# jhbastek/PhysicsInformedDiffusionModels

Measured on NVIDIA H100. Metric: train samples/s Darcy 64x64 PIDM, higher is better.
Workload: dtype bf16

## Files before the change

include/pidm.h:

```cpp
#ifndef PIDM_H_
#define PIDM_H_

#ifdef __cplusplus
extern "C" {
#endif

#ifndef PIDM_F32
#define PIDM_F32 0
#define PIDM_BF16 1
#endif

const char* pidm_last_error(void);
int pidm_version(void);

int pidm_qsample(const float* x0, const float* noise, const long long* t, const float* sqrt_ab,
                 const float* sqrt_1mab, float* xt, int B, int per_sample, void* stream);
int pidm_posterior_step(const float* x_t, const float* x0_pred, const float* z, float* out, float coef1, float coef2,
                        float sigma, long long n, void* stream);
int pidm_axpby_per_sample(const float* a, const float* x, const float* b, const float* y, const float* c,
                          const float* z, float* out, int B, int per_sample, void* stream);
int pidm_ddim_coefs(const long long* t, const long long* t_next, const float* posterior_mean_coef1,
                    const float* posterior_mean_coef2, const float* sqrt_recip_alphas, const float* noise_mean_coeff,
                    const float* alphas_prod, float* coef_x0, float* coef_x, int B, void* stream);
int pidm_scale(const float* x, const float* alpha_dev, float* out, long long n, void* stream);

int pidm_toy_pidm_loss(const float* target, const float* output, const float* residual, const float* ineq,
                       const float* opt, const long long* t, const float* p2_loss_weight,
                       const float* posterior_var_clipped, float c_data, float c_residual, float c_ineq, float lambda_opt,
                       float* sums7, float* grad_output, float* grad_residual, float* grad_ineq, float* grad_opt, int B,
                       int D, void* stream);

#define PIDM_DARCY_PIXELS_AT_BOUNDARY 1
#define PIDM_DARCY_PERIODIC 2
int pidm_darcy_residual_fwd(const float* x0hat, const float* f_s, float* residual, int B, int pixels,
                            float domain_length, int reverse_d1, int flags, void* stream);
int pidm_darcy_residual_bwd(const float* x0hat, const float* f_s, const float* grad_residual, float* grad_x0hat, int B,
                            int pixels, float domain_length, int reverse_d1, int flags, void* stream);
#define PIDM_FD_PERIODIC 8
int pidm_fd_stencil(const float* u, float* out, int planes, int pixels, int mode, float d0, float d1, void* stream);
int pidm_darcy_pidm_loss(const float* x0hat, const float* model_out, const float* target, const float* f_s,
                         const long long* t, const float* p2_loss_weight, const float* posterior_var_clipped,
                         float c_data, float c_residual, float* sums3, float* grad_x0hat, float* grad_model_out, int B,
                         int pixels, float domain_length, int reverse_d1, int flags, void* stream);
int pidm_darcy_jacobian_max(const float* x0hat, float* max_dr_dp, int B, int pixels, float domain_length, int reverse_d1,
                            int flags, void* stream);

int pidm_nchw_to_nhwc(const float* src, void* dst, int B, int C, int HW, int Cpad, int dtype, void* stream);
int pidm_nhwc_to_nchw(const void* src, float* dst, int B, int C, int HW, int Cpad, int dtype, void* stream);
int pidm_add(const void* a, const void* b, void* out, long long n, int dtype, void* stream);
int pidm_gelu_fwd(const void* x, void* y, long long n, int dtype, void* stream);
int pidm_gelu_bwd(const void* x, const void* dy, void* dx, long long n, int dtype, void* stream);
int pidm_concat_channels(const void* a, const void* b, void* out, long long rows, int Ca, int Cb, int dtype, void* stream);
int pidm_split_channels(const void* g, void* ga, void* gb, long long rows, int Ca, int Cb, int dtype, void* stream);

int pidm_pack_entry_size(void);
int pidm_pack_weights(const void* table_dev, int n_entries, int dtype, void* stream);
int pidm_pack_pair_entry_size(void);
int pidm_pack_weights_pairs(const void* table_dev, const int* tile_map_dev, int tile_base, int n_tiles, int max_taps,
                            int dtype, void* stream);
int pidm_conv2d_simt(const void* x, const void* w_packed, const float* bias, const void* residual, void* y, int B,
                     int H, int W, int Cin, int Ho, int Wo, int Cout, int KH, int KW, int stride, int pad,
                     int transposed, int dtype, void* stream);
int pidm_conv2d_wgrad_simt(const void* x, const void* dy, float* dw, float* dbias, int B, int H, int W, int Cin,
                           int Cin_real, int Ho, int Wo, int Cout, int KH, int KW, int stride, int pad, int transposed,
                           long long w_stride_n, long long w_stride_c, int dtype, void* stream);
int pidm_debug_set_trace(void* buf);
int pidm_conv2d_tc_general(const void* x, const void* w_packed, const float* bias, const void* residual, void* y, int B,
                           int H, int W, int Cin, int Ho, int Wo, int Cout, int KH, int KW, int stride, int pad,
                           int transposed, float* gn_sums, int gn_groups, int gn_sums_zeroed, void* stream);
int pidm_conv2d_tc_general_supported(int B, int H, int W, int Cin, int Ho, int Wo, int Cout, int KH, int KW, int stride,
                                     int pad, int transposed);
int pidm_conv2d_tc_plan(int B, int H, int W, int Cin, int Ho, int Wo, int Cout, int KH, int KW, int stride, int pad,
                        int transposed, int* out);
int pidm_conv2d_wgrad_tc(const void* a, const void* b, float* dw, int B, int HA, int WA, int CA, int CA_real, int GH,
                         int GW, int CB, int KH, int KW, int a_stride, int pad, long long s_row, long long s_col,
                         void* stream);
int pidm_conv2d_wgrad_tc_supported(int B, int GH, int GW, int CA, int CB, int KH, int KW, int a_stride);
int pidm_conv2d_wgrad_tc_plan(int B, int HA, int WA, int CA, int CA_real, int GH, int GW, int CB, int KH, int KW,
                              int a_stride, int pad, long long s_row, long long s_col, int* out);
int pidm_colsum(const void* x, float* out, long long M, int C, int dtype, void* stream);

int pidm_groupnorm_silu_fwd(const void* x, const float* gamma, const float* beta, const float* scale_shift,
                            const void* residual, void* y, float* sums, int stats_precomputed, int B, int HW, int C, int G,
                            float eps, int dtype, void* stream);
int pidm_groupnorm_silu_bwd(const void* x, const void* dy, const float* sums, const float* gamma, const float* beta,
                            const float* scale_shift, void* dx, float* dgamma, float* dbeta, float* d_scale_shift,
                            float* dbias_of_producer, float* workspace, int B, int HW, int C, int G, float eps,
                            int dtype, void* stream);
int pidm_layernorm_c_fwd(const void* x, const float* gamma, void* y, long long M, int C, float eps, int dtype, void* stream);
int pidm_layernorm_c_bwd(const void* x, const void* dy, const float* gamma, void* dx, float* dgamma,
                         const void* dx_residual , long long M, int C,
                         float eps, int dtype, void* stream);

int pidm_linattn_fused_supported(int C, int heads, int N, int dtype);
int pidm_linattn_fused_workspace_floats(int B, int N);
int pidm_linattn_fused_plan(int B, int N, int* out);
int pidm_linattn_fused_fwd(const void* xn, const void* w_qkv, void* out, float* ctx, float* kmax, float* kzinv,
                           float* workspace, int B, int N, void* stream);
int pidm_linattn_fused_bwd(const void* xn, const void* w_qkv, const void* dout, const float* ctx, const float* kmax,
                           const float* kzinv, void* dxn, float* dctx, int B, int N, void* stream);
int pidm_linattn_fused_wgrad(const void* xn, const void* w_qkv, const void* dout, const float* ctx, const float* dctx,
                             const float* kmax, const float* kzinv, float* grad_w, int B, int N, long long w_stride_n,
                             long long w_stride_c, void* stream);
int pidm_linattn_workspace_floats(int B, int N, int heads);
int pidm_linattn_fwd(const void* qkv, void* out, float* ctx, float* kmax, float* kzinv, float* workspace, int B, int N,
                     int heads, int dtype, void* stream);
int pidm_linattn_bwd(const void* qkv, const void* dout, const float* ctx, const float* kmax, const float* kzinv,
                     void* dqkv, float* dctx_scratch, int B, int N, int heads, int dtype, void* stream);
int pidm_attn_fwd(const void* qkv, void* out, int B, int n_tokens, int heads, int dtype, void* stream);
int pidm_attn_bwd(const void* qkv, const void* dout, void* dqkv, int B, int n_tokens, int heads, int dtype, void* stream);

int pidm_time_embed_fwd(const long long* t, const float* W1, const float* b1, const float* W2, const float* b2,
                        float* emb, float* h1, float* temb, float* silu_t, int B, int dim, int td, void* stream);
int pidm_time_embed_bwd(const float* d_silu_t, const float* emb, const float* h1, const float* temb, const float* W2,
                        float* dW1, float* db1, float* dW2, float* db2, float* workspace, int B, int dim, int td,
                        int parts, void* stream);
int pidm_mlp_entry_size(void);
int pidm_block_mlps_fwd(const void* table_dev, int n_entries, int max_rows, const float* silu_t, int B, int td,
                        void* stream);
int pidm_block_mlps_bwd(const void* table_dev, int n_entries, int max_rows, const float* silu_t, float* d_silu_t, int B,
                        int td, int parts, void* stream);

int pidm_head_fwd(const void* x, const float* w, const float* bias, float* y, int B, int HW, int C, int O,
                  int sigmoid_last, int dtype, void* stream);
int pidm_head_bwd(const void* x, const float* w, const float* y, const float* dy, void* dx, float* dw, float* db, int B,
                  int HW, int C, int O, int sigmoid_last, int dtype, void* stream);

int pidm_sumsq(const float* x, long long n, float* out, float* workspace, void* stream);
int pidm_adam_ema_step(float* param, float* grad, float* exp_avg, float* exp_avg_sq, float* ema_shadow, long long n,
                       float lr, double beta1, double beta2, float eps, int step, int* step_counter_dev,
                       const float* grad_norm_sq_dev, float grad_scale, float max_norm, float ema_mu,
                       int ema_first_step, int zero_grad, void* stream);

int pidm_mechanics_residual_fwd(const float* u, const float* rho, const float* bcs, const float* KE, float* residual,
                                float* compliance, int B, int nel, void* stream);
int pidm_mechanics_residual_bwd(const float* u, const float* rho, const float* bcs, const float* KE,
                                const float* grad_residual, const float* grad_compliance, float* grad_u, float* grad_rho,
                                float* workspace , int B, int nel, void* stream);
int pidm_mech_pidm_loss(const float* u, const float* rho, const float* x0, const float* residual, const float* compliance,
                        const float* vf, const long long* t, const float* p2_loss_weight,
                        const float* posterior_var_clipped, float c_data, float c_residual, float c_ineq,
                        float lambda_opt, float* sums6, float* grad_u, float* grad_rho, float* grad_residual,
                        float* grad_compliance, int B, int nel, void* stream);
int pidm_bilinear_resize_fwd(const float* x, float* y, int planes, int in, int out, void* stream);
int pidm_bilinear_resize_bwd(const float* dy, float* dx, int planes, int in, int out, void* stream);

#ifdef __cplusplus
}
#endif
#endif
```

physicsinformeddiffusionmodels_b200/_lib.py:

```python
import ctypes
import os

import torch

_HERE = os.path.dirname(os.path.abspath(__file__))
LIB_PATH = os.path.join(_HERE, 'libpidm.so')

P = ctypes.c_void_p
I = ctypes.c_int
L = ctypes.c_longlong
F = ctypes.c_float
D = ctypes.c_double

_SIGS = {
    'pidm_qsample': [P, P, P, P, P, P, I, I, P],
    'pidm_posterior_step': [P, P, P, P, F, F, F, L, P],
    'pidm_scale': [P, P, P, L, P],
    'pidm_ddim_coefs': [P, P, P, P, P, P, P, P, P, I, P],
    'pidm_axpby_per_sample': [P, P, P, P, P, P, P, I, I, P],
    'pidm_toy_pidm_loss': [P, P, P, P, P, P, P, P, F, F, F, F, P, P, P, P, P, I, I, P],
    'pidm_fd_stencil': [P, P, I, I, I, F, F, P],
    'pidm_darcy_residual_fwd': [P, P, P, I, I, F, I, I, P],
    'pidm_darcy_residual_bwd': [P, P, P, P, I, I, F, I, I, P],
    'pidm_darcy_jacobian_max': [P, P, I, I, F, I, I, P],
    'pidm_darcy_pidm_loss': [P, P, P, P, P, P, P, F, F, P, P, P, I, I, F, I, I, P],
    'pidm_nchw_to_nhwc': [P, P, I, I, I, I, I, P],
    'pidm_nhwc_to_nchw': [P, P, I, I, I, I, I, P],
    'pidm_add': [P, P, P, L, I, P],
    'pidm_gelu_fwd': [P, P, L, I, P],
    'pidm_gelu_bwd': [P, P, P, L, I, P],
    'pidm_concat_channels': [P, P, P, L, I, I, I, P],
    'pidm_split_channels': [P, P, P, L, I, I, I, P],
    'pidm_pack_entry_size': [],
    'pidm_pack_weights': [P, I, I, P],
    'pidm_pack_pair_entry_size': [],
    'pidm_pack_weights_pairs': [P, P, I, I, I, I, P],
    'pidm_conv2d_simt': [P, P, P, P, P, I, I, I, I, I, I, I, I, I, I, I, I, I, P],
    'pidm_conv2d_wgrad_simt': [P, P, P, P, I, I, I, I, I, I, I, I, I, I, I, I, I, L, L, I, P],
    'pidm_debug_set_trace': [P],
    'pidm_conv2d_tc_general': [P, P, P, P, P, I, I, I, I, I, I, I, I, I, I, I, I, P, I, I, P],
    'pidm_conv2d_tc_general_supported': [I, I, I, I, I, I, I, I, I, I, I, I],
    'pidm_conv2d_tc_plan': [I, I, I, I, I, I, I, I, I, I, I, I, P],
    'pidm_conv2d_wgrad_tc': [P, P, P, I, I, I, I, I, I, I, I, I, I, I, I, L, L, P],
    'pidm_conv2d_wgrad_tc_supported': [I, I, I, I, I, I, I, I],
    'pidm_conv2d_wgrad_tc_plan': [I, I, I, I, I, I, I, I, I, I, I, I, L, L, P],
    'pidm_colsum': [P, P, L, I, I, P],
    'pidm_groupnorm_silu_fwd': [P, P, P, P, P, P, P, I, I, I, I, I, F, I, P],
    'pidm_groupnorm_silu_bwd': [P, P, P, P, P, P, P, P, P, P, P, P, I, I, I, I, F, I, P],
    'pidm_layernorm_c_fwd': [P, P, P, L, I, F, I, P],
    'pidm_layernorm_c_bwd': [P, P, P, P, P, P, L, I, F, I, P],
    'pidm_linattn_workspace_floats': [I, I, I],
    'pidm_linattn_fused_supported': [I, I, I, I],
    'pidm_linattn_fused_workspace_floats': [I, I],
    'pidm_linattn_fused_plan': [I, I, P],
    'pidm_linattn_fused_fwd': [P, P, P, P, P, P, P, I, I, P],
    'pidm_linattn_fused_bwd': [P, P, P, P, P, P, P, P, I, I, P],
    'pidm_linattn_fused_wgrad': [P, P, P, P, P, P, P, P, I, I, L, L, P],
    'pidm_linattn_fwd': [P, P, P, P, P, P, I, I, I, I, P],
    'pidm_linattn_bwd': [P, P, P, P, P, P, P, I, I, I, I, P],
    'pidm_attn_fwd': [P, P, I, I, I, I, P],
    'pidm_attn_bwd': [P, P, P, I, I, I, I, P],
    'pidm_time_embed_fwd': [P, P, P, P, P, P, P, P, P, I, I, I, P],
    'pidm_time_embed_bwd': [P, P, P, P, P, P, P, P, P, P, I, I, I, I, P],
    'pidm_mlp_entry_size': [],
    'pidm_block_mlps_fwd': [P, I, I, P, I, I, P],
    'pidm_block_mlps_bwd': [P, I, I, P, P, I, I, I, P],
    'pidm_head_fwd': [P, P, P, P, I, I, I, I, I, I, P],
    'pidm_head_bwd': [P, P, P, P, P, P, P, I, I, I, I, I, I, P],
    'pidm_sumsq': [P, L, P, P, P],
    'pidm_adam_ema_step': [P, P, P, P, P, L, F, D, D, F, I, P, P, F, F, F, I, I, P],
    'pidm_mechanics_residual_fwd': [P, P, P, P, P, P, I, I, P],
    'pidm_mechanics_residual_bwd': [P, P, P, P, P, P, P, P, P, I, I, P],
    'pidm_mech_pidm_loss': [P, P, P, P, P, P, P, P, P, F, F, F, F, P, P, P, P, P, I, I, P],
    'pidm_bilinear_resize_fwd': [P, P, I, I, I, P],
    'pidm_bilinear_resize_bwd': [P, P, I, I, I, P],
    'pidm_version': [],
}
_VALUE_RETURN = {'pidm_pack_entry_size', 'pidm_pack_pair_entry_size', 'pidm_mlp_entry_size', 'pidm_linattn_workspace_floats', 'pidm_version',
                 'pidm_linattn_fused_supported', 'pidm_linattn_fused_workspace_floats',
                 'pidm_conv2d_tc_supported', 'pidm_conv2d_wgrad_tc_supported', 'pidm_conv2d_tc_general_supported',
                 'pidm_conv2d_tc_plan', 'pidm_conv2d_wgrad_tc_plan', 'pidm_linattn_fused_plan'}

if not os.path.exists(LIB_PATH):
    raise ImportError(f'{LIB_PATH} is missing: build it with `python __graft_entry__.py` (nvcc, sm_90a). '
                      'There is no CPU / PyTorch fallback for the PIDM hot path.')

_lib = ctypes.CDLL(LIB_PATH)
_lib.pidm_last_error.restype = ctypes.c_char_p
_lib.pidm_last_error.argtypes = []
for _n, _a in _SIGS.items():
    _f = getattr(_lib, _n)
    _f.argtypes = _a
    _f.restype = ctypes.c_int

launch_count = 0


def exported_symbols():
    return sorted(_SIGS) + ['pidm_last_error']


def ptr(t):
    if t is None:
        return None
    return t.data_ptr()


def stream():
    return torch.cuda.current_stream().cuda_stream


def call(name, *args):
    global launch_count
    conv = []
    for a in args:
        if isinstance(a, torch.Tensor):
            conv.append(a.data_ptr())
        else:
            conv.append(a)
    rc = getattr(_lib, name)(*conv)
    if name in _VALUE_RETURN:
        return rc
    launch_count += 1
    if rc != 0:
        raise RuntimeError(f'{name} failed (code {rc}): {_lib.pidm_last_error().decode()}')
    return 0


DTYPE_CODE = {torch.float32: 0, torch.bfloat16: 1}
```

physicsinformeddiffusionmodels_b200/csrc/attention_fused.cu:

```cuda
#define PIDM_PDL_GROUP 1
#include "common.cuh"
#include "mma_util.cuh"
#include "pidm.h"

namespace pidm {

constexpr int LF_C = 32;

__device__ __forceinline__ uint32_t movm_t(uint32_t x) {
    uint32_t y;
    asm volatile("movmatrix.sync.aligned.m8n8.trans.b16 %0, %1;" : "=r"(y) : "r"(x));
    return y;
}

__device__ __forceinline__ void load_w_frags(uint32_t (&w)[2][4][2], const __nv_bfloat16* __restrict__ Wrows, int lane) {
    const int g = lane >> 2, t = lane & 3;
#pragma unroll
    for (int ks = 0; ks < 2; ++ks)
#pragma unroll
        for (int nt = 0; nt < 4; ++nt) {
            const uint32_t* row = reinterpret_cast<const uint32_t*>(Wrows + (size_t)(nt * 8 + g) * LF_C + ks * 16 + 2 * t);
            w[ks][nt][0] = __ldg(row);
            w[ks][nt][1] = __ldg(row + 4);
        }
}
template <int MT>
__device__ __forceinline__ void load_x_frags(uint32_t (&a)[MT][2][4], const __nv_bfloat16* Xs, int lane) {
#pragma unroll
    for (int mt = 0; mt < MT; ++mt)
#pragma unroll
        for (int ks = 0; ks < 2; ++ks) frag_a_rowmajor(a[mt][ks], Xs, LW_PITCH, mt * 16, ks * 16, lane);
}
template <int MT>
__device__ __forceinline__ void project(float (&c)[MT][4][4], const uint32_t (&a)[MT][2][4], const uint32_t (&w)[2][4][2]) {
#pragma unroll
    for (int mt = 0; mt < MT; ++mt)
#pragma unroll
        for (int nt = 0; nt < 4; ++nt) {
#pragma unroll
            for (int i = 0; i < 4; ++i) c[mt][nt][i] = 0.f;
#pragma unroll
            for (int ks = 0; ks < 2; ++ks) mma_bf16(c[mt][nt], a[mt][ks], w[ks][nt][0], w[ks][nt][1]);
        }
}
__device__ __forceinline__ void frag_softmax(float (&c)[4][4], float mul) {
#pragma unroll
    for (int half = 0; half < 2; ++half) {
        float mx = -INFINITY;
#pragma unroll
        for (int nt = 0; nt < 4; ++nt) mx = fmaxf(mx, fmaxf(c[nt][half * 2], c[nt][half * 2 + 1]));
        mx = fmaxf(mx, __shfl_xor_sync(0xffffffffu, mx, 1));
        mx = fmaxf(mx, __shfl_xor_sync(0xffffffffu, mx, 2));
        float s = 0.f;
#pragma unroll
        for (int nt = 0; nt < 4; ++nt) {
            c[nt][half * 2] = __expf(c[nt][half * 2] - mx);
            c[nt][half * 2 + 1] = __expf(c[nt][half * 2 + 1] - mx);
            s += c[nt][half * 2] + c[nt][half * 2 + 1];
        }
        s += __shfl_xor_sync(0xffffffffu, s, 1);
        s += __shfl_xor_sync(0xffffffffu, s, 2);
        const float inv = mul / s;
#pragma unroll
        for (int nt = 0; nt < 4; ++nt) { c[nt][half * 2] *= inv; c[nt][half * 2 + 1] *= inv; }
    }
}
__device__ __forceinline__ void c_to_a(uint32_t (&a)[2][4], const float (&c)[4][4]) {
#pragma unroll
    for (int ks = 0; ks < 2; ++ks) {
        a[ks][0] = pack_bf16(c[2 * ks][0], c[2 * ks][1]);
        a[ks][1] = pack_bf16(c[2 * ks][2], c[2 * ks][3]);
        a[ks][2] = pack_bf16(c[2 * ks + 1][0], c[2 * ks + 1][1]);
        a[ks][3] = pack_bf16(c[2 * ks + 1][2], c[2 * ks + 1][3]);
    }
}
__device__ __forceinline__ void load_cols(float (&v)[8], const float* __restrict__ src, int lane) {
    const int t = lane & 3;
#pragma unroll
    for (int nt = 0; nt < 4; ++nt) { v[nt * 2] = src[nt * 8 + 2 * t]; v[nt * 2 + 1] = src[nt * 8 + 2 * t + 1]; }
}

constexpr int LFS_STAGES = 2;
__global__ void __launch_bounds__(256) laf_kmax_kernel(const __nv_bfloat16* __restrict__ xn,
                                                       const __nv_bfloat16* __restrict__ W, float* __restrict__ part,
                                                       int N, int rows_per_chunk) {
    pdl_trigger();
    pdl_wait();
    extern __shared__ __align__(16) unsigned char raw[];
    const int b = blockIdx.y, chunk = blockIdx.x, lane = threadIdx.x & 31, h = threadIdx.x >> 5;
    __nv_bfloat16* ring = reinterpret_cast<__nv_bfloat16*>(raw) + (size_t)h * (LFS_STAGES * LW_TILE);
    const int n_begin = chunk * rows_per_chunk, n_end = min(N, n_begin + rows_per_chunk);
    const int n_tiles = (n_end - n_begin) / 32;
    const __nv_bfloat16* xsrc = xn + ((size_t)b * N + n_begin) * LF_C;
    auto issue = [&](int it) {
        if (it < n_tiles) lw_issue<32>(ring + (size_t)(it % LFS_STAGES) * LW_TILE, xsrc + (size_t)it * 32 * LF_C, LF_C, lane);
        cp_commit();
    };
#pragma unroll
    for (int s = 0; s < LFS_STAGES; ++s) issue(s);
    uint32_t wk[2][4][2];
    load_w_frags(wk, W + (size_t)(LM_HID + h * LM_D) * LF_C, lane);
    float m[8];
#pragma unroll
    for (int i = 0; i < 8; ++i) m[i] = -INFINITY;
    for (int it = 0; it < n_tiles; ++it) {
        cp_wait<LFS_STAGES - 1>();
        __syncwarp();
        uint32_t ax[2][2][4];
        load_x_frags<2>(ax, ring + (size_t)(it % LFS_STAGES) * LW_TILE, lane);
        __syncwarp();
        issue(it + LFS_STAGES);
        float ck[2][4][4];
        project<2>(ck, ax, wk);
#pragma unroll
        for (int nt = 0; nt < 4; ++nt)
#pragma unroll
            for (int j = 0; j < 2; ++j)
                m[nt * 2 + j] = fmaxf(fmaxf(m[nt * 2 + j], fmaxf(ck[0][nt][j], ck[0][nt][2 + j])),
                                      fmaxf(ck[1][nt][j], ck[1][nt][2 + j]));
    }
#pragma unroll
    for (int off = 4; off < 32; off <<= 1)
#pragma unroll
        for (int i = 0; i < 8; ++i) m[i] = fmaxf(m[i], __shfl_xor_sync(0xffffffffu, m[i], off));
    if (lane < 4) {
        float* o = part + ((size_t)b * gridDim.x + chunk) * LM_HID + h * LM_D;
#pragma unroll
        for (int nt = 0; nt < 4; ++nt)
#pragma unroll
            for (int j = 0; j < 2; ++j) o[nt * 8 + 2 * lane + j] = m[nt * 2 + j];
    }
}

__global__ void laf_finalize_kernel(float* __restrict__ ctx, float* __restrict__ kzinv, int n_rows) {
    pdl_trigger();
    pdl_wait();
    const int row = blockIdx.x * (blockDim.x / 32) + (threadIdx.x >> 5), lane = threadIdx.x & 31;
    if (row >= n_rows) return;
    const float zi = 1.f / kzinv[row];
    ctx[(size_t)row * LM_D + lane] *= zi;
    __syncwarp();
    if (lane == 0) kzinv[row] = zi;
}

template <int MODE>
struct LfcCfg {
    static constexpr int STAGES = MODE == 0 ? 4 : 2;
    static constexpr int STAGE_ELEMS = MODE == 0 ? LW_TILE : 2 * LW_TILE;
    static constexpr size_t SMEM = (size_t)LM_HEADS * STAGES * STAGE_ELEMS * 2 + (size_t)LM_HEADS * 2 * LM_D * 4;
};
template <int MODE>
__global__ void __launch_bounds__(256, 2) laf_ctx_kernel(const __nv_bfloat16* __restrict__ xn, const __nv_bfloat16* __restrict__ W,
                                                      const __nv_bfloat16* __restrict__ dout, const float* __restrict__ part,
                                                      int n_stat_chunks, float* __restrict__ kmax, float* __restrict__ kzinv,
                                                      float* __restrict__ ctx, int N, int chunk_px, float scale) {
    pdl_trigger();
    pdl_wait();
    extern __shared__ __align__(16) unsigned char raw[];
    constexpr int LFC_STAGES = LfcCfg<MODE>::STAGES, LFC_STAGE_ELEMS = LfcCfg<MODE>::STAGE_ELEMS;
    const int b = blockIdx.y, chunk = blockIdx.x, lane = threadIdx.x & 31, h = threadIdx.x >> 5;
    __nv_bfloat16* ring = reinterpret_cast<__nv_bfloat16*>(raw) + (size_t)h * (LFC_STAGES * LFC_STAGE_ELEMS);
    float* sM = reinterpret_cast<float*>(raw + (size_t)LM_HEADS * LFC_STAGES * LFC_STAGE_ELEMS * 2) + h * 2 * LM_D;
    float* sZi = sM + LM_D;
    const int n_begin = chunk * chunk_px, n_end = min(N, n_begin + chunk_px);
    const int n_tiles = (n_end - n_begin) / 32;
    const size_t pix0 = (size_t)b * N + n_begin;
    const __nv_bfloat16* xsrc = xn + pix0 * LF_C;
    const __nv_bfloat16* gsrc = (MODE == 1) ? dout + pix0 * LM_HID + h * LM_D : nullptr;
    auto issue = [&](int it) {
        if (it < n_tiles) {
            __nv_bfloat16* buf = ring + (size_t)(it % LFC_STAGES) * LFC_STAGE_ELEMS;
            lw_issue<32>(buf, xsrc + (size_t)it * 32 * LF_C, LF_C, lane);
            if (MODE == 1) lw_issue<32>(buf + LW_TILE, gsrc + (size_t)it * 32 * LM_HID, LM_HID, lane);
        }
        cp_commit();
    };
#pragma unroll
    for (int s = 0; s < LFC_STAGES; ++s) issue(s);
    uint32_t w0[2][4][2], w1[2][4][2];
    load_w_frags(w0, W + (size_t)((MODE == 0 ? LM_HID : 0) + h * LM_D) * LF_C, lane);
    if (MODE == 0) load_w_frags(w1, W + (size_t)(2 * LM_HID + h * LM_D) * LF_C, lane);
    float Mc[8];
    float zacc[8];
#pragma unroll
    for (int i = 0; i < 8; ++i) zacc[i] = 0.f;
    if (MODE == 0) {
        const int c = h * LM_D + lane;
        float M = -INFINITY;
        for (int i = 0; i < n_stat_chunks; ++i) M = fmaxf(M, part[((size_t)b * n_stat_chunks + i) * LM_HID + c]);
        sM[lane] = M;
        if (chunk == 0) kmax[(size_t)b * LM_HID + c] = M;
        __syncwarp();
        load_cols(Mc, sM, lane);
    }
    float acc[2][4][4];
#pragma unroll
    for (int i = 0; i < 2; ++i)
#pragma unroll
        for (int j = 0; j < 4; ++j)
#pragma unroll
            for (int k = 0; k < 4; ++k) acc[i][j][k] = 0.f;
    for (int it = 0; it < n_tiles; ++it) {
        cp_wait<LFC_STAGES - 1>();
        __syncwarp();
        const __nv_bfloat16* buf = ring + (size_t)(it % LFC_STAGES) * LFC_STAGE_ELEMS;
        uint32_t ax[2][2][4];
        load_x_frags<2>(ax, buf, lane);
        uint32_t bv[2][4][2];
        if (MODE == 1) {
#pragma unroll
            for (int ks = 0; ks < 2; ++ks) {
                uint32_t b01[4], b23[4];
                frag_b_krows(b01, buf + LW_TILE, LW_PITCH, ks * 16, 0, lane);
                frag_b_krows(b23, buf + LW_TILE, LW_PITCH, ks * 16, 16, lane);
                bv[ks][0][0] = b01[0]; bv[ks][0][1] = b01[1]; bv[ks][1][0] = b01[2]; bv[ks][1][1] = b01[3];
                bv[ks][2][0] = b23[0]; bv[ks][2][1] = b23[1]; bv[ks][3][0] = b23[2]; bv[ks][3][1] = b23[3];
            }
        }
        __syncwarp();
        issue(it + LFC_STAGES);
        float cw[2][4][4];
        project<2>(cw, ax, w0);
        if (MODE == 0) {
#pragma unroll
            for (int mt = 0; mt < 2; ++mt)
#pragma unroll
                for (int nt = 0; nt < 4; ++nt)
#pragma unroll
                    for (int i = 0; i < 4; ++i) {
                        cw[mt][nt][i] = __expf(cw[mt][nt][i] - Mc[nt * 2 + (i & 1)]);
                        zacc[nt * 2 + (i & 1)] += cw[mt][nt][i];
                    }
            float cv[2][4][4];
            project<2>(cv, ax, w1);
#pragma unroll
            for (int mt = 0; mt < 2; ++mt)
#pragma unroll
                for (int nt = 0; nt < 4; ++nt) {
                    bv[mt][nt][0] = movm_t(pack_bf16(cv[mt][nt][0], cv[mt][nt][1]));
                    bv[mt][nt][1] = movm_t(pack_bf16(cv[mt][nt][2], cv[mt][nt][3]));
                }
        } else {
            frag_softmax(cw[0], scale);
            frag_softmax(cw[1], scale);
        }
#pragma unroll
        for (int mt = 0; mt < 2; ++mt) {
#pragma unroll
            for (int md = 0; md < 2; ++md) {
                uint32_t a[4];
                a[0] = movm_t(pack_bf16(cw[mt][2 * md][0], cw[mt][2 * md][1]));
                a[1] = movm_t(pack_bf16(cw[mt][2 * md + 1][0], cw[mt][2 * md + 1][1]));
                a[2] = movm_t(pack_bf16(cw[mt][2 * md][2], cw[mt][2 * md][3]));
                a[3] = movm_t(pack_bf16(cw[mt][2 * md + 1][2], cw[mt][2 * md + 1][3]));
#pragma unroll
                for (int ne = 0; ne < 4; ++ne) mma_bf16(acc[md][ne], a, bv[mt][ne][0], bv[mt][ne][1]);
            }
        }
    }
    const int g = lane >> 2, t = lane & 3;
    if (MODE == 0) {
#pragma unroll
        for (int off = 4; off < 32; off <<= 1)
#pragma unroll
            for (int i = 0; i < 8; ++i) zacc[i] += __shfl_xor_sync(0xffffffffu, zacc[i], off);
        if (lane < 4) {
#pragma unroll
            for (int nt = 0; nt < 4; ++nt)
#pragma unroll
                for (int j = 0; j < 2; ++j)
                    atomicAdd(kzinv + (size_t)b * LM_HID + h * LM_D + nt * 8 + 2 * lane + j, zacc[nt * 2 + j]);
        }
    }
    float* cb = ctx + ((size_t)b * LM_HEADS + h) * LM_D * LM_D;
#pragma unroll
    for (int md = 0; md < 2; ++md)
#pragma unroll
        for (int half = 0; half < 2; ++half) {
            const int d = md * 16 + g + half * 8;
            const float f = (MODE == 0) ? 1.f / (float)N : 1.f;
#pragma unroll
            for (int ne = 0; ne < 4; ++ne) {
                const int e = ne * 8 + 2 * t;
                atomicAdd(cb + d * LM_D + e, acc[md][ne][half * 2] * f);
                atomicAdd(cb + d * LM_D + e + 1, acc[md][ne][half * 2 + 1] * f);
            }
        }
}

constexpr int LFO_STAGES = 2;
__global__ void __launch_bounds__(256) laf_out_kernel(const __nv_bfloat16* __restrict__ xn, const __nv_bfloat16* __restrict__ W,
                                                      const float* __restrict__ ctx, __nv_bfloat16* __restrict__ out, int N,
                                                      int chunk_px, float scale) {
    pdl_trigger();
    pdl_wait();
    extern __shared__ __align__(16) unsigned char raw[];
    const int b = blockIdx.y, chunk = blockIdx.x, lane = threadIdx.x & 31, h = threadIdx.x >> 5;
    __nv_bfloat16* ring = reinterpret_cast<__nv_bfloat16*>(raw) + (size_t)h * ((LFO_STAGES + 1) * LW_TILE);
    __nv_bfloat16* Os = ring + LFO_STAGES * LW_TILE;
    const int n_begin = chunk * chunk_px, n_end = min(N, n_begin + chunk_px);
    const int n_tiles = (n_end - n_begin) / 32;
    const size_t pix0 = (size_t)b * N + n_begin;
    const __nv_bfloat16* xsrc = xn + pix0 * LF_C;
    __nv_bfloat16* odst = out + pix0 * LM_HID + h * LM_D;
    auto issue = [&](int it) {
        if (it < n_tiles) lw_issue<32>(ring + (size_t)(it % LFO_STAGES) * LW_TILE, xsrc + (size_t)it * 32 * LF_C, LF_C, lane);
        cp_commit();
    };
#pragma unroll
    for (int s = 0; s < LFO_STAGES; ++s) issue(s);
    uint32_t wq[2][4][2];
    load_w_frags(wq, W + (size_t)(h * LM_D) * LF_C, lane);
    const float* ch = ctx + ((size_t)b * LM_HEADS + h) * LM_D * LM_D;
    uint32_t bf[2][4][2];
#pragma unroll
    for (int ks = 0; ks < 2; ++ks)
#pragma unroll
        for (int nt = 0; nt < 4; ++nt) frag_b_global<true>(bf[ks][nt], ch, ks * 16, nt * 8, lane);
    const int g = lane >> 2, t = lane & 3;
    for (int it = 0; it < n_tiles; ++it) {
        cp_wait<LFO_STAGES - 1>();
        __syncwarp();
        uint32_t ax[2][2][4];
        load_x_frags<2>(ax, ring + (size_t)(it % LFO_STAGES) * LW_TILE, lane);
        __syncwarp();
        issue(it + LFO_STAGES);
        float cq[2][4][4];
        project<2>(cq, ax, wq);
#pragma unroll
        for (int mt = 0; mt < 2; ++mt) {
            frag_softmax(cq[mt], scale);
            uint32_t a[2][4];
            c_to_a(a, cq[mt]);
            float c[4][4];
#pragma unroll
            for (int i = 0; i < 4; ++i)
#pragma unroll
                for (int k = 0; k < 4; ++k) c[i][k] = 0.f;
#pragma unroll
            for (int ks = 0; ks < 2; ++ks)
#pragma unroll
                for (int nt = 0; nt < 4; ++nt) mma_bf16(c[nt], a[ks], bf[ks][nt][0], bf[ks][nt][1]);
#pragma unroll
            for (int nt = 0; nt < 4; ++nt) {
                __nv_bfloat16* o = Os + (size_t)(mt * 16 + g) * LW_PITCH + nt * 8 + 2 * t;
                *reinterpret_cast<uint32_t*>(o) = pack_bf16(c[nt][0], c[nt][1]);
                *reinterpret_cast<uint32_t*>(o + 8 * LW_PITCH) = pack_bf16(c[nt][2], c[nt][3]);
            }
        }
        __syncwarp();
        lw_store<32>(odst + (size_t)it * 32 * LM_HID, LM_HID, Os, lane);
        __syncwarp();
    }
}

constexpr int LFB_ROWS = 16;
constexpr int LFB_STAGES = 4;
constexpr int LFB_TILE = LFB_ROWS * LW_PITCH;

struct LfbTile {
    uint32_t ax[1][2][4], ag[2][4];
};
__device__ __forceinline__ void lfb_dq(float (&dq)[4][4], const LfbTile& tl, const uint32_t (&wq)[2][4][2],
                                       const uint32_t (&bc)[2][4][2], float scale) {
    float c1[1][4][4], c2[4][4];
    project<1>(c1, tl.ax, wq);
    frag_softmax(c1[0], 1.f);
#pragma unroll
    for (int nt = 0; nt < 4; ++nt) {
#pragma unroll
        for (int i = 0; i < 4; ++i) c2[nt][i] = 0.f;
#pragma unroll
        for (int ks = 0; ks < 2; ++ks) mma_bf16(c2[nt], tl.ag[ks], bc[ks][nt][0], bc[ks][nt][1]);
    }
#pragma unroll
    for (int half = 0; half < 2; ++half) {
        float dot = 0.f;
#pragma unroll
        for (int nt = 0; nt < 4; ++nt)
            dot += c1[0][nt][half * 2] * c2[nt][half * 2] + c1[0][nt][half * 2 + 1] * c2[nt][half * 2 + 1];
        dot += __shfl_xor_sync(0xffffffffu, dot, 1);
        dot += __shfl_xor_sync(0xffffffffu, dot, 2);
#pragma unroll
        for (int nt = 0; nt < 4; ++nt)
#pragma unroll
            for (int j = 0; j < 2; ++j) dq[nt][half * 2 + j] = scale * c1[0][nt][half * 2 + j] * (c2[nt][half * 2 + j] - dot);
    }
}
__device__ __forceinline__ void lfb_dkdv(float (&dk)[4][4], float (&dv)[4][4], const uint32_t (&ax)[1][2][4],
                                         const uint32_t (&wk)[2][4][2], const uint32_t (&wv)[2][4][2],
                                         const uint32_t (&bd)[2][4][2], const uint32_t (&bt)[2][4][2],
                                         const float (&Mc)[8], const float (&Zc)[8], const float (&cdc)[8], float invN) {
    float c1[1][4][4];
    uint32_t a[2][4];
    project<1>(c1, ax, wv);
    c_to_a(a, c1[0]);
#pragma unroll
    for (int nt = 0; nt < 4; ++nt) {
#pragma unroll
        for (int i = 0; i < 4; ++i) dk[nt][i] = 0.f;
#pragma unroll
        for (int ks = 0; ks < 2; ++ks) mma_bf16(dk[nt], a[ks], bd[ks][nt][0], bd[ks][nt][1]);
    }
    project<1>(c1, ax, wk);
#pragma unroll
    for (int nt = 0; nt < 4; ++nt)
#pragma unroll
        for (int i = 0; i < 4; ++i) {
            c1[0][nt][i] = __expf(c1[0][nt][i] - Mc[nt * 2 + (i & 1)]) * Zc[nt * 2 + (i & 1)];
            dk[nt][i] = c1[0][nt][i] * (dk[nt][i] * invN - cdc[nt * 2 + (i & 1)]);
        }
    c_to_a(a, c1[0]);
#pragma unroll
    for (int nt = 0; nt < 4; ++nt) {
#pragma unroll
        for (int i = 0; i < 4; ++i) dv[nt][i] = 0.f;
#pragma unroll
        for (int ks = 0; ks < 2; ++ks) mma_bf16(dv[nt], a[ks], bt[ks][nt][0], bt[ks][nt][1]);
#pragma unroll
        for (int i = 0; i < 4; ++i) dv[nt][i] *= invN;
    }
}
__device__ __forceinline__ void lfb_cd(float (&cdc)[8], float* scd, const float* __restrict__ cg, const float* __restrict__ dg,
                                       int lane) {
    float s = 0.f;
#pragma unroll
    for (int e = 0; e < LM_D; e += 4) {
        const float4 x = *reinterpret_cast<const float4*>(dg + lane * LM_D + e);
        const float4 y = *reinterpret_cast<const float4*>(cg + lane * LM_D + e);
        s += x.x * y.x + x.y * y.y + x.z * y.z + x.w * y.w;
    }
    scd[lane] = s;
    __syncwarp();
    load_cols(cdc, scd, lane);
}

constexpr int LFB_STAGE_ELEMS = (1 + LM_HEADS) * LFB_TILE;
constexpr int LFB_W_PITCH = LF_C + 8;
constexpr int LFB_R_PITCH = LF_C + 8;
constexpr size_t LAF_BWD_SMEM = (size_t)LFB_STAGES * LFB_STAGE_ELEMS * 2 + (size_t)3 * LM_HID * LFB_W_PITCH * 2 +
                                (size_t)LM_HEADS * LFB_ROWS * LFB_R_PITCH * 4 + (size_t)LM_HEADS * LM_D * 4;

__device__ __forceinline__ void mma_w(float (&c)[4][4], const uint32_t (&g)[2][4], const __nv_bfloat16* Wh, int lane) {
#pragma unroll
    for (int kd = 0; kd < 2; ++kd)
#pragma unroll
        for (int np = 0; np < 2; ++np) {
            uint32_t bw[4];
            frag_b_krows(bw, Wh, LFB_W_PITCH, kd * 16, np * 16, lane);
            mma_bf16(c[2 * np], g[kd], bw[0], bw[1]);
            mma_bf16(c[2 * np + 1], g[kd], bw[2], bw[3]);
        }
}

__global__ void __launch_bounds__(256) laf_bwd_kernel(const __nv_bfloat16* __restrict__ xn, const __nv_bfloat16* __restrict__ W,
                                                      const __nv_bfloat16* __restrict__ dout, const float* __restrict__ ctx,
                                                      const float* __restrict__ dctx, const float* __restrict__ kmax,
                                                      const float* __restrict__ kzinv, __nv_bfloat16* __restrict__ dxn,
                                                      int N, int chunk_px, float scale) {
    pdl_trigger();
    pdl_wait();
    extern __shared__ __align__(16) unsigned char raw[];
    const int b = blockIdx.y, chunk = blockIdx.x, lane = threadIdx.x & 31, h = threadIdx.x >> 5;
    __nv_bfloat16* ring = reinterpret_cast<__nv_bfloat16*>(raw);
    __nv_bfloat16* Ws = ring + LFB_STAGES * LFB_STAGE_ELEMS;
    float* R = reinterpret_cast<float*>(Ws + 3 * LM_HID * LFB_W_PITCH);
    float* scd = R + LM_HEADS * LFB_ROWS * LFB_R_PITCH + h * LM_D;
    const int n_begin = chunk * chunk_px, n_end = min(N, n_begin + chunk_px);
    const int n_tiles = (n_end - n_begin) / LFB_ROWS;
    const size_t pix0 = (size_t)b * N + n_begin;
    const __nv_bfloat16* xsrc = xn + pix0 * LF_C;
    const __nv_bfloat16* gsrc = dout + pix0 * LM_HID + h * LM_D;
    for (int i = threadIdx.x; i < 3 * LM_HID * (LF_C / 8); i += blockDim.x)
        cp_async16(Ws + (i >> 2) * LFB_W_PITCH + (i & 3) * 8, W + (size_t)(i >> 2) * LF_C + (i & 3) * 8);
    cp_commit();
    auto issue = [&](int it) {
        if (it < n_tiles) {
            __nv_bfloat16* buf = ring + (size_t)(it % LFB_STAGES) * LFB_STAGE_ELEMS;
            if (h == 0) lw_issue<LFB_ROWS>(buf, xsrc + (size_t)it * LFB_ROWS * LF_C, LF_C, lane);
            lw_issue<LFB_ROWS>(buf + (1 + h) * LFB_TILE, gsrc + (size_t)it * LFB_ROWS * LM_HID, LM_HID, lane);
        }
        cp_commit();
    };
#pragma unroll
    for (int s = 0; s < LFB_STAGES - 1; ++s) issue(s);
    const float* cg = ctx + ((size_t)b * LM_HEADS + h) * LM_D * LM_D;
    const float* dg = dctx + ((size_t)b * LM_HEADS + h) * LM_D * LM_D;
    float Mc[8], Zc[8], cdc[8];
    lfb_cd(cdc, scd, cg, dg, lane);
    load_cols(Mc, kmax + (size_t)b * LM_HID + h * LM_D, lane);
    load_cols(Zc, kzinv + (size_t)b * LM_HID + h * LM_D, lane);
    uint32_t wq[2][4][2], wk[2][4][2], wv[2][4][2];
    load_w_frags(wq, W + (size_t)(h * LM_D) * LF_C, lane);
    load_w_frags(wk, W + (size_t)(LM_HID + h * LM_D) * LF_C, lane);
    load_w_frags(wv, W + (size_t)(2 * LM_HID + h * LM_D) * LF_C, lane);
    uint32_t bc[2][4][2], bd[2][4][2], bt[2][4][2];
#pragma unroll
    for (int ks = 0; ks < 2; ++ks)
#pragma unroll
        for (int nt = 0; nt < 4; ++nt) {
            frag_b_global<false>(bc[ks][nt], cg, ks * 16, nt * 8, lane);
            frag_b_global<false>(bd[ks][nt], dg, ks * 16, nt * 8, lane);
            frag_b_global<true>(bt[ks][nt], dg, ks * 16, nt * 8, lane);
        }
    const int g = lane >> 2, t = lane & 3;
    const float invN = 1.f / (float)N;
    const __nv_bfloat16* Wq = Ws + (size_t)(h * LM_D) * LFB_W_PITCH;
    const __nv_bfloat16* Wk = Wq + (size_t)LM_HID * LFB_W_PITCH;
    const __nv_bfloat16* Wv = Wk + (size_t)LM_HID * LFB_W_PITCH;
    float* Rw = R + h * LFB_ROWS * LFB_R_PITCH;
    const int rrow = threadIdx.x >> 4, rcol = (threadIdx.x & 15) * 2;
    for (int it = 0; it < n_tiles; ++it) {
        cp_wait<LFB_STAGES - 2>();
        __syncthreads();
        issue(it + LFB_STAGES - 1);
        const __nv_bfloat16* buf = ring + (size_t)(it % LFB_STAGES) * LFB_STAGE_ELEMS;
        LfbTile tl;
        load_x_frags<1>(tl.ax, buf, lane);
        frag_a_rowmajor(tl.ag[0], buf + (1 + h) * LFB_TILE, LW_PITCH, 0, 0, lane);
        frag_a_rowmajor(tl.ag[1], buf + (1 + h) * LFB_TILE, LW_PITCH, 0, 16, lane);
        float dx[4][4];
#pragma unroll
        for (int nt = 0; nt < 4; ++nt)
#pragma unroll
            for (int i = 0; i < 4; ++i) dx[nt][i] = 0.f;
        uint32_t a[2][4];
        {
            float dq[4][4];
            lfb_dq(dq, tl, wq, bc, scale);
            c_to_a(a, dq);
            mma_w(dx, a, Wq, lane);
        }
        {
            float dk[4][4], dv[4][4];
            lfb_dkdv(dk, dv, tl.ax, wk, wv, bd, bt, Mc, Zc, cdc, invN);
            c_to_a(a, dk);
            mma_w(dx, a, Wk, lane);
            c_to_a(a, dv);
            mma_w(dx, a, Wv, lane);
        }
#pragma unroll
        for (int nt = 0; nt < 4; ++nt)
#pragma unroll
            for (int half = 0; half < 2; ++half)
                *reinterpret_cast<float2*>(Rw + (g + half * 8) * LFB_R_PITCH + nt * 8 + 2 * t) =
                    make_float2(dx[nt][half * 2], dx[nt][half * 2 + 1]);
        __syncthreads();
        float sx = 0.f, sy = 0.f;
#pragma unroll
        for (int w = 0; w < LM_HEADS; ++w) {
            const float2 v = *reinterpret_cast<const float2*>(R + (w * LFB_ROWS + rrow) * LFB_R_PITCH + rcol);
            sx += v.x;
            sy += v.y;
        }
        *reinterpret_cast<uint32_t*>(dxn + (pix0 + (size_t)it * LFB_ROWS + rrow) * LF_C + rcol) = pack_bf16(sx, sy);
    }
}

template <int PART>
struct LfwCfg {
    static constexpr int MATS = PART == 0 ? 1 : 2;
    static constexpr int STAGE_ELEMS = (PART == 0 ? 2 : 1) * LFB_TILE;
    static constexpr int S_PITCH = LM_D + 1;
    static_assert(LFB_STAGES * STAGE_ELEMS * 2 >= LM_D * S_PITCH * 4, "the epilogue staging reuses the tile ring");
    static constexpr size_t SMEM = (size_t)LM_HEADS * (LFB_STAGES * STAGE_ELEMS * 2 + LM_D * 4);
};

__device__ __forceinline__ void acc_gtx(float (&acc)[2][4][4], const float (&gf)[4][4], const uint32_t (&bx)[2][4]) {
#pragma unroll
    for (int md = 0; md < 2; ++md) {
        uint32_t a[4];
        a[0] = movm_t(pack_bf16(gf[2 * md][0], gf[2 * md][1]));
        a[1] = movm_t(pack_bf16(gf[2 * md + 1][0], gf[2 * md + 1][1]));
        a[2] = movm_t(pack_bf16(gf[2 * md][2], gf[2 * md][3]));
        a[3] = movm_t(pack_bf16(gf[2 * md + 1][2], gf[2 * md + 1][3]));
#pragma unroll
        for (int np = 0; np < 2; ++np) {
            mma_bf16(acc[md][2 * np], a, bx[np][0], bx[np][1]);
            mma_bf16(acc[md][2 * np + 1], a, bx[np][2], bx[np][3]);
        }
    }
}

template <int PART>
__global__ void __launch_bounds__(256) laf_wgrad_kernel(const __nv_bfloat16* __restrict__ xn, const __nv_bfloat16* __restrict__ W,
                                                        const __nv_bfloat16* __restrict__ dout, const float* __restrict__ ctx,
                                                        const float* __restrict__ dctx, const float* __restrict__ kmax,
                                                        const float* __restrict__ kzinv, float* __restrict__ grad_w, int N,
                                                        int chunk_px, long long w_stride_n, long long w_stride_c, float scale) {
    pdl_trigger();
    pdl_wait();
    extern __shared__ __align__(16) unsigned char raw[];
    constexpr int MATS = LfwCfg<PART>::MATS, STAGE_ELEMS = LfwCfg<PART>::STAGE_ELEMS, S_PITCH = LfwCfg<PART>::S_PITCH;
    const int b = blockIdx.y, chunk = blockIdx.x, lane = threadIdx.x & 31, h = threadIdx.x >> 5;
    __nv_bfloat16* ring = reinterpret_cast<__nv_bfloat16*>(raw) + (size_t)h * (LFB_STAGES * STAGE_ELEMS);
    float* scd = reinterpret_cast<float*>(raw + (size_t)LM_HEADS * LFB_STAGES * STAGE_ELEMS * 2) + h * LM_D;
    const int n_begin = chunk * chunk_px, n_end = min(N, n_begin + chunk_px);
    const int n_tiles = (n_end - n_begin) / LFB_ROWS;
    const size_t pix0 = (size_t)b * N + n_begin;
    const __nv_bfloat16* xsrc = xn + pix0 * LF_C;
    const __nv_bfloat16* gsrc = dout + pix0 * LM_HID + h * LM_D;
    auto issue = [&](int it) {
        if (it < n_tiles) {
            __nv_bfloat16* buf = ring + (size_t)(it % LFB_STAGES) * STAGE_ELEMS;
            lw_issue<LFB_ROWS>(buf, xsrc + (size_t)it * LFB_ROWS * LF_C, LF_C, lane);
            if (PART == 0) lw_issue<LFB_ROWS>(buf + LFB_TILE, gsrc + (size_t)it * LFB_ROWS * LM_HID, LM_HID, lane);
        }
        cp_commit();
    };
#pragma unroll
    for (int s = 0; s < LFB_STAGES; ++s) issue(s);
    const float* cg = ctx + ((size_t)b * LM_HEADS + h) * LM_D * LM_D;
    const float* dg = dctx + ((size_t)b * LM_HEADS + h) * LM_D * LM_D;
    float Mc[8], Zc[8], cdc[8];
    uint32_t w0[2][4][2], w1[2][4][2];
    uint32_t b0[2][4][2], b1[2][4][2];
    if (PART == 0) {
        load_w_frags(w0, W + (size_t)(h * LM_D) * LF_C, lane);
    } else {
        lfb_cd(cdc, scd, cg, dg, lane);
        load_cols(Mc, kmax + (size_t)b * LM_HID + h * LM_D, lane);
        load_cols(Zc, kzinv + (size_t)b * LM_HID + h * LM_D, lane);
        load_w_frags(w0, W + (size_t)(LM_HID + h * LM_D) * LF_C, lane);
        load_w_frags(w1, W + (size_t)(2 * LM_HID + h * LM_D) * LF_C, lane);
    }
#pragma unroll
    for (int ks = 0; ks < 2; ++ks)
#pragma unroll
        for (int nt = 0; nt < 4; ++nt) {
            frag_b_global<false>(b0[ks][nt], PART == 0 ? cg : dg, ks * 16, nt * 8, lane);
            if (PART == 1) frag_b_global<true>(b1[ks][nt], dg, ks * 16, nt * 8, lane);
        }
    const float invN = 1.f / (float)N;
    float acc[MATS][2][4][4];
#pragma unroll
    for (int m = 0; m < MATS; ++m)
#pragma unroll
        for (int i = 0; i < 2; ++i)
#pragma unroll
            for (int j = 0; j < 4; ++j)
#pragma unroll
                for (int k = 0; k < 4; ++k) acc[m][i][j][k] = 0.f;
    for (int it = 0; it < n_tiles; ++it) {
        cp_wait<LFB_STAGES - 1>();
        __syncwarp();
        const __nv_bfloat16* buf = ring + (size_t)(it % LFB_STAGES) * STAGE_ELEMS;
        LfbTile tl;
        load_x_frags<1>(tl.ax, buf, lane);
        uint32_t bx[2][4];
        frag_b_krows(bx[0], buf, LW_PITCH, 0, 0, lane);
        frag_b_krows(bx[1], buf, LW_PITCH, 0, 16, lane);
        if (PART == 0) {
            frag_a_rowmajor(tl.ag[0], buf + LFB_TILE, LW_PITCH, 0, 0, lane);
            frag_a_rowmajor(tl.ag[1], buf + LFB_TILE, LW_PITCH, 0, 16, lane);
        }
        __syncwarp();
        issue(it + LFB_STAGES);
        if (PART == 0) {
            float dq[4][4];
            lfb_dq(dq, tl, w0, b0, scale);
            acc_gtx(acc[0], dq, bx);
        } else {
            float dk[4][4], dv[4][4];
            lfb_dkdv(dk, dv, tl.ax, w0, w1, b0, b1, Mc, Zc, cdc, invN);
            acc_gtx(acc[0], dk, bx);
            acc_gtx(acc[MATS - 1], dv, bx);
        }
    }
    cp_wait<0>();
    __syncwarp();
    float* S = reinterpret_cast<float*>(ring);
    const int g = lane >> 2, t = lane & 3;
#pragma unroll
    for (int m = 0; m < MATS; ++m) {
#pragma unroll
        for (int md = 0; md < 2; ++md)
#pragma unroll
            for (int nc = 0; nc < 4; ++nc)
#pragma unroll
                for (int i = 0; i < 4; ++i) S[(md * 16 + g + 8 * (i >> 1)) * S_PITCH + nc * 8 + 2 * t + (i & 1)] = acc[m][md][nc][i];
        __syncwarp();
        float* dst = grad_w + (long long)((PART + m) * LM_HID + h * LM_D) * w_stride_n + lane * w_stride_c;
#pragma unroll 4
        for (int d = 0; d < LM_D; ++d) atomicAdd(dst + d * w_stride_n, S[d * S_PITCH + lane]);
        __syncwarp();
    }
}

constexpr size_t LAF_STATS_SMEM = (size_t)LM_HEADS * LFS_STAGES * LW_TILE * 2;
constexpr size_t LAF_OUT_SMEM = (size_t)LM_HEADS * (LFO_STAGES + 1) * LW_TILE * 2;

static int laf_attrs() {
    static bool done = false;
    if (!done) {
        PIDM_CUDA(cudaFuncSetAttribute(laf_kmax_kernel, cudaFuncAttributeMaxDynamicSharedMemorySize, (int)LAF_STATS_SMEM));
        PIDM_CUDA(cudaFuncSetAttribute(laf_ctx_kernel<0>, cudaFuncAttributeMaxDynamicSharedMemorySize, (int)LfcCfg<0>::SMEM));
        PIDM_CUDA(cudaFuncSetAttribute(laf_ctx_kernel<1>, cudaFuncAttributeMaxDynamicSharedMemorySize, (int)LfcCfg<1>::SMEM));
        PIDM_CUDA(cudaFuncSetAttribute(laf_out_kernel, cudaFuncAttributeMaxDynamicSharedMemorySize, (int)LAF_OUT_SMEM));
        PIDM_CUDA(cudaFuncSetAttribute(laf_bwd_kernel, cudaFuncAttributeMaxDynamicSharedMemorySize, (int)LAF_BWD_SMEM));
        PIDM_CUDA(cudaFuncSetAttribute(laf_wgrad_kernel<0>, cudaFuncAttributeMaxDynamicSharedMemorySize, (int)LfwCfg<0>::SMEM));
        PIDM_CUDA(cudaFuncSetAttribute(laf_wgrad_kernel<1>, cudaFuncAttributeMaxDynamicSharedMemorySize, (int)LfwCfg<1>::SMEM));
        done = true;
    }
    return 0;
}

static int laf_chunk_px(int B, int N, int ctas_per_sm) {
    int k = (num_sms() * ctas_per_sm) / B;
    if (k < 1) k = 1;
    int px = ((N + k - 1) / k + 31) / 32 * 32;
    if (px < 64) px = 64;
    if (px > N) px = N;
    return px;
}
static int laf_stat_chunks(int N) {
    int c = N / 128;
    if (c < 1) c = 1;
    if (c > 16) c = 16;
    return c;
}

}
using namespace pidm;

extern "C" int pidm_linattn_fused_supported(int C, int heads, int N, int dtype) {
    return (C == LF_C && heads == LM_HEADS && dtype == PIDM_BF16 && N % 128 == 0) ? 1 : 0;
}

extern "C" int pidm_linattn_fused_workspace_floats(int B, int N) { return B * laf_stat_chunks(N) * LM_HID; }

extern "C" int pidm_linattn_fused_plan(int B, int N, int* out) {
    PIDM_REQUIRE(N % 128 == 0 && B > 0, "linattn_fused_plan: N must be a multiple of 128 (got %d)", N);
    const int v[5] = {laf_stat_chunks(N), laf_chunk_px(B, N, 2), laf_chunk_px(B, N, 3), laf_chunk_px(B, N, 1),
                      laf_chunk_px(B, N, 1)};
    for (int i = 0; i < 5; ++i) out[i] = v[i];
    return 0;
}

extern "C" int pidm_linattn_fused_fwd(const void* xn, const void* w_qkv, void* out, float* ctx, float* kmax, float* kzinv,
                                      float* workspace, int B, int N, void* stream) {
    PIDM_REQUIRE(N % 128 == 0, "linattn_fused: N must be a multiple of 128 (got %d)", N);
    cudaStream_t st = (cudaStream_t)stream;
    if (int e = laf_attrs()) return e;
    const float scale = 0.17677669529663687f;
    const __nv_bfloat16* x = (const __nv_bfloat16*)xn;
    const __nv_bfloat16* w = (const __nv_bfloat16*)w_qkv;
    PIDM_CUDA(cudaMemsetAsync(ctx, 0, (size_t)B * LM_HEADS * LM_D * LM_D * sizeof(float), st));
    PIDM_CUDA(cudaMemsetAsync(kzinv, 0, (size_t)B * LM_HID * sizeof(float), st));
    const int chunks = laf_stat_chunks(N);
    const int rpc = N / chunks;
    PIDM_REQUIRE(rpc % 32 == 0 && rpc * chunks == N, "linattn_fused: bad statistics chunking for N=%d", N);
    PIDM_CUDA(launch_pdl(laf_kmax_kernel, dim3(dim3(chunks, B)), dim3(256), (size_t)(LAF_STATS_SMEM), st, x, w, workspace, N, rpc));
    const int cpx = laf_chunk_px(B, N, 2);
    PIDM_CUDA(launch_pdl(laf_ctx_kernel<0>, dim3(dim3((N + cpx - 1) / cpx, B)), dim3(256), (size_t)(LfcCfg<0>::SMEM), st, x, w, nullptr, workspace, chunks, kmax, kzinv,
                                                                             ctx, N, cpx, scale));
    PIDM_CUDA(launch_pdl(laf_finalize_kernel, dim3((B * LM_HID + 7) / 8), dim3(256), (size_t)(0), st, ctx, kzinv, B * LM_HID));
    const int opx = laf_chunk_px(B, N, 3);
    PIDM_CUDA(launch_pdl(laf_out_kernel, dim3(dim3((N + opx - 1) / opx, B)), dim3(256), (size_t)(LAF_OUT_SMEM), st, x, w, ctx, (__nv_bfloat16*)out, N, opx, scale));
    PIDM_LAUNCH_CHECK("linattn_fused_fwd");
    return 0;
}

extern "C" int pidm_linattn_fused_bwd(const void* xn, const void* w_qkv, const void* dout, const float* ctx,
                                      const float* kmax, const float* kzinv, void* dxn, float* dctx, int B, int N,
                                      void* stream) {
    PIDM_REQUIRE(N % 128 == 0, "linattn_fused: N must be a multiple of 128 (got %d)", N);
    cudaStream_t st = (cudaStream_t)stream;
    if (int e = laf_attrs()) return e;
    const float scale = 0.17677669529663687f;
    const __nv_bfloat16* x = (const __nv_bfloat16*)xn;
    const __nv_bfloat16* w = (const __nv_bfloat16*)w_qkv;
    PIDM_CUDA(cudaMemsetAsync(dctx, 0, (size_t)B * LM_HEADS * LM_D * LM_D * sizeof(float), st));
    const int cpx = laf_chunk_px(B, N, 2);
    PIDM_CUDA(launch_pdl(laf_ctx_kernel<1>, dim3(dim3((N + cpx - 1) / cpx, B)), dim3(256), (size_t)(LfcCfg<1>::SMEM), st, x, w, (const __nv_bfloat16*)dout, nullptr, 0,
                                                                             nullptr, nullptr, dctx, N, cpx, scale));
    const int bpx = laf_chunk_px(B, N, 1);
    PIDM_CUDA(launch_pdl(laf_bwd_kernel, dim3(dim3((N + bpx - 1) / bpx, B)), dim3(256), (size_t)(LAF_BWD_SMEM), st, x, w, (const __nv_bfloat16*)dout, ctx, dctx, kmax,
                                                                          kzinv, (__nv_bfloat16*)dxn, N, bpx, scale));
    PIDM_LAUNCH_CHECK("linattn_fused_bwd");
    return 0;
}

extern "C" int pidm_linattn_fused_wgrad(const void* xn, const void* w_qkv, const void* dout, const float* ctx,
                                        const float* dctx, const float* kmax, const float* kzinv, float* grad_w, int B,
                                        int N, long long w_stride_n, long long w_stride_c, void* stream) {
    PIDM_REQUIRE(N % 128 == 0, "linattn_fused: N must be a multiple of 128 (got %d)", N);
    cudaStream_t st = (cudaStream_t)stream;
    if (int e = laf_attrs()) return e;
    const float scale = 0.17677669529663687f;
    const __nv_bfloat16* x = (const __nv_bfloat16*)xn;
    const __nv_bfloat16* w = (const __nv_bfloat16*)w_qkv;
    const __nv_bfloat16* g = (const __nv_bfloat16*)dout;
    const int px = laf_chunk_px(B, N, 1);
    const dim3 grid((N + px - 1) / px, B);
    PIDM_CUDA(launch_pdl(laf_wgrad_kernel<0>, grid, dim3(256), LfwCfg<0>::SMEM, st, x, w, g, ctx, dctx, kmax, kzinv, grad_w, N,
                         px, w_stride_n, w_stride_c, scale));
    PIDM_CUDA(launch_pdl(laf_wgrad_kernel<1>, grid, dim3(256), LfwCfg<1>::SMEM, st, x, w, g, ctx, dctx, kmax, kzinv, grad_w, N,
                         px, w_stride_n, w_stride_c, scale));
    PIDM_LAUNCH_CHECK("linattn_fused_wgrad");
    return 0;
}
```

physicsinformeddiffusionmodels_b200/ops.py:

```python
import os

import torch

from . import _lib
from ._lib import call, stream

_TC_HARD_OFF = os.environ.get('PIDM_DISABLE_TC') == '1'
_STATE = {'act_dtype': torch.bfloat16, 'use_tc': not _TC_HARD_OFF}


def set_precision(name):
    _STATE['act_dtype'] = {'bf16': torch.bfloat16, 'fp32': torch.float32}[name]


def set_tensor_core_conv(flag):
    _STATE['use_tc'] = bool(flag) and not _TC_HARD_OFF


def act_dtype():
    return _STATE['act_dtype']


def _code(t):
    return _lib.DTYPE_CODE[t.dtype]


def _grad_buffer(p):
    g = getattr(p, '_pidm_grad', None)
    if g is not None:
        return g, None
    z = torch.zeros_like(p)
    return z, z


def _need_cuda(*ts):
    for t in ts:
        if t is not None and not t.is_cuda:
            raise RuntimeError('physicsinformeddiffusionmodels_b200 runs on CUDA (H100) only: got a CPU tensor. '
                               'There is no CPU fallback on the product path.')


def _need_f32(**named):
    for k, t in named.items():
        if t is None:
            continue
        if not t.is_cuda:
            raise RuntimeError(f'{k}: expected a CUDA tensor (no CPU fallback on the product path)')
        if t.dtype != torch.float32 or not t.is_contiguous():
            raise RuntimeError(f'{k}: expected a contiguous float32 tensor, got {t.dtype}, strides {t.stride()}')


def nchw_to_nhwc(x, cpad, dtype=None):
    _need_cuda(x)
    B, C, H, W = x.shape
    dtype = dtype or act_dtype()
    y = torch.empty(B, H, W, cpad, device=x.device, dtype=dtype)
    call('pidm_nchw_to_nhwc', x.contiguous().float(), y, B, C, H * W, cpad, _lib.DTYPE_CODE[dtype], stream())
    return y


def nhwc_to_nchw(x, C=None):
    B, H, W, Cp = x.shape
    C = C or Cp
    y = torch.empty(B, C, H, W, device=x.device, dtype=torch.float32)
    call('pidm_nhwc_to_nchw', x, y, B, C, H * W, Cp, _code(x), stream())
    return y


class _Add(torch.autograd.Function):
    @staticmethod
    def forward(ctx, a, b):
        o = torch.empty_like(a)
        call('pidm_add', a, b, o, a.numel(), _code(a), stream())
        return o

    @staticmethod
    def backward(ctx, g):
        return g, g


def add(a, b):
    return _Add.apply(a.contiguous(), b.contiguous())


class _Gelu(torch.autograd.Function):
    @staticmethod
    def forward(ctx, x):
        y = torch.empty_like(x)
        call('pidm_gelu_fwd', x, y, x.numel(), _code(x), stream())
        ctx.save_for_backward(x)
        return y

    @staticmethod
    def backward(ctx, dy):
        (x,) = ctx.saved_tensors
        dx = torch.empty_like(x)
        call('pidm_gelu_bwd', x, dy.contiguous(), dx, x.numel(), _code(x), stream())
        return dx


def gelu(x):
    return _Gelu.apply(x.contiguous())


class _Stash(torch.autograd.Function):

    @staticmethod
    def forward(ctx, x, link):
        ctx.link = link
        link['expect_skip'] = True
        return x.view_as(x)

    @staticmethod
    def backward(ctx, g):
        ctx.link['skip'] = g.contiguous()
        return None, None


def stash_grad(x, link):
    return _Stash.apply(x, link)


def _take_skip(link):
    if link is None or not link.get('expect_skip'):
        return None
    if 'skip' not in link:
        raise RuntimeError('skip-connection gradient was expected but has not been produced yet (autograd order)')
    return link.pop('skip')


class _Concat(torch.autograd.Function):
    @staticmethod
    def forward(ctx, a, b):
        B, H, W, Ca = a.shape
        Cb = b.shape[-1]
        o = torch.empty(B, H, W, Ca + Cb, device=a.device, dtype=a.dtype)
        call('pidm_concat_channels', a, b, o, B * H * W, Ca, Cb, _code(a), stream())
        ctx.shapes = (a.shape, b.shape)
        return o

    @staticmethod
    def backward(ctx, g):
        sa, sb = ctx.shapes
        g = g.contiguous()
        ga = torch.empty(sa, device=g.device, dtype=g.dtype)
        gb = torch.empty(sb, device=g.device, dtype=g.dtype)
        call('pidm_split_channels', g, ga, gb, sa[0] * sa[1] * sa[2], sa[3], sb[3], _code(g), stream())
        return ga, gb


def concat(a, b):
    return _Concat.apply(a.contiguous(), b.contiguous())


_ZERO_POOL = {'buf': None, 'cur': 0}


def zero_pool_begin(nfloats, device):
    _ZERO_POOL['buf'] = torch.zeros(int(nfloats), device=device, dtype=torch.float32)
    _ZERO_POOL['cur'] = 0


def zero_pool_end():
    _ZERO_POOL['buf'] = None


def _zero_take(*shape):
    buf = _ZERO_POOL['buf']
    n = 1
    for d in shape:
        n *= int(d)
    n_al = (n + 31) // 32 * 32
    if buf is None or _ZERO_POOL['cur'] + n_al > buf.numel():
        return None
    out = buf[_ZERO_POOL['cur']:_ZERO_POOL['cur'] + n].view(*shape)
    _ZERO_POOL['cur'] += n_al
    return out


def _conv_launch(x, wp, bias, residual, y, g, transposed, gn_sums=None, gn_groups=0, gn_zeroed=False):
    B, H, W, Cin, Ho, Wo, Cout, KH, KW, stride, pad = g
    tr = 1 if transposed else 0
    if (_STATE['use_tc'] and x.dtype == torch.bfloat16
            and call('pidm_conv2d_tc_general_supported', B, H, W, Cin, Ho, Wo, Cout, KH, KW, stride, pad, tr)):
        cpg = Cout // gn_groups if gn_groups else 0
        fuse = gn_sums is not None and (cpg in (4, 8, 16) or (cpg > 0 and cpg % 32 == 0))
        call('pidm_conv2d_tc_general', x, wp, bias, residual, y, B, H, W, Cin, Ho, Wo, Cout, KH, KW, stride, pad, tr,
             gn_sums if fuse else None, gn_groups if fuse else 0, 1 if gn_zeroed else 0, stream())
        return fuse
    else:
        call('pidm_conv2d_simt', x, wp, bias, residual, y, B, H, W, Cin, Ho, Wo, Cout, KH, KW, stride, pad,
             1 if transposed else 0, _code(x), stream())
        return False


class _Conv2d(torch.autograd.Function):

    @staticmethod
    def forward(ctx, x, weight, bias, residual, spec, link, skip):
        B, H, W, Cin = x.shape
        Ho, Wo = spec.out_hw(H, W)
        y = torch.empty(B, Ho, Wo, spec.cout, device=x.device, dtype=x.dtype)
        g = (B, H, W, Cin, Ho, Wo, spec.cout, spec.kh, spec.kw, spec.stride, spec.pad)
        sums, zeroed = None, False
        if link is not None:
            sums = _zero_take(B, link['groups'], 2)
            zeroed = sums is not None
            if sums is None:
                sums = torch.empty(B, link['groups'], 2, device=x.device, dtype=torch.float32)
        fused = _conv_launch(x, spec.wp_fwd, bias, residual, y, g, spec.transposed, sums, link['groups'] if link else 0,
                             zeroed)
        if link is not None:
            link['sums'] = sums if fused else None
            link['bias'] = bias
        ctx.save_for_backward(x, weight, bias)
        ctx.spec, ctx.g, ctx.has_res, ctx.link, ctx.skip = spec, g, residual is not None, link, skip
        if skip is not None and skip[0] == 'park':
            skip[1]['expect_skip'] = True
        return y

    @staticmethod
    def backward(ctx, dy):
        x, weight, bias = ctx.saved_tensors
        dy = dy.contiguous()
        skip = ctx.skip
        dgrad_res = _take_skip(skip[1]) if (skip is not None and skip[0] == 'take' and ctx.needs_input_grad[0]) else None
        dx, gw_ret, gb_ret = _conv_backward(x, weight, bias, ctx.spec, ctx.g, dy, ctx.needs_input_grad[0], ctx.link,
                                            dgrad_res)
        if skip is not None and skip[0] == 'park':
            skip[1]['skip'] = dx
            dx = None
        return dx, gw_ret, gb_ret, (dy if ctx.has_res else None), None, None, None


_SIDE = {'streams': [], 'next': 0, 'keep': [], 'active': False}
_N_SIDE = max(1, int(os.environ.get('PIDM_SIDE_STREAMS', '1')))


def side_stream_begin():
    if os.environ.get('PIDM_NO_SIDE_STREAM') == '1':
        return
    while len(_SIDE['streams']) < _N_SIDE:
        _SIDE['streams'].append(torch.cuda.Stream())
    _SIDE['active'] = True
    _SIDE['next'] = 0
    _SIDE['keep'] = []


def side_stream_join():
    if _SIDE['active']:
        for st in _SIDE['streams']:
            torch.cuda.current_stream().wait_stream(st)
        _SIDE['keep'] = []
        _SIDE['active'] = False


_FORK = {'stream': None}


def fork_stream():
    if _FORK['stream'] is None:
        _FORK['stream'] = torch.cuda.Stream()
    _FORK['stream'].wait_stream(torch.cuda.current_stream())
    return _FORK['stream']


def _wgrad_stream(*operands):
    if not _SIDE['active']:
        return stream()
    side = _SIDE['streams'][_SIDE['next']]
    _SIDE['next'] = (_SIDE['next'] + 1) % len(_SIDE['streams'])
    side.wait_stream(torch.cuda.current_stream())
    _SIDE['keep'].extend(operands)
    return side.cuda_stream


def _conv_backward(x, weight, bias, spec, g, dy, need_dx, link=None, dgrad_residual=None):
    B, H, W, Cin, Ho, Wo, Cout, KH, KW, stride, pad = g
    dx = None
    if need_dx or dgrad_residual is not None:
        dx = torch.empty_like(x)
        if stride == 1 and not spec.transposed:
            gd = (B, Ho, Wo, Cout, H, W, Cin, KH, KW, 1, KH - 1 - pad)
            _conv_launch(dy, spec.wp_dgrad, None, dgrad_residual, dx, gd, False)
        else:
            gd = (B, Ho, Wo, Cout, H, W, Cin, KH, KW, stride, pad)
            _conv_launch(dy, spec.wp_dgrad, None, dgrad_residual, dx, gd, not spec.transposed)
    gw_buf, gw_ret = _grad_buffer(weight)
    gb_buf, gb_ret = (None, None) if bias is None else _grad_buffer(bias)
    if link is not None and 'dbias' in link:
        gb_buf, gb_ret = None, link.pop('dbias')
    use_tc = _STATE['use_tc'] and x.dtype == torch.bfloat16
    ws = _wgrad_stream(x, dy)
    if use_tc and not spec.transposed and call('pidm_conv2d_wgrad_tc_supported', B, Ho, Wo, Cin, Cout, KH, KW, stride):
        call('pidm_conv2d_wgrad_tc', x, dy, gw_buf, B, H, W, Cin, spec.cin_real, Ho, Wo, Cout, KH, KW, stride, pad,
             spec.w_stride_c, spec.w_stride_n, ws)
        if gb_buf is not None:
            call('pidm_colsum', dy, gb_buf, B * Ho * Wo, Cout, _code(dy), ws)
    elif use_tc and spec.transposed and call('pidm_conv2d_wgrad_tc_supported', B, H, W, Cout, Cin, KH, KW, stride):
        call('pidm_conv2d_wgrad_tc', dy, x, gw_buf, B, Ho, Wo, Cout, Cout, H, W, Cin, KH, KW, stride, pad,
             spec.w_stride_n, spec.w_stride_c, ws)
        if gb_buf is not None:
            call('pidm_colsum', dy, gb_buf, B * Ho * Wo, Cout, _code(dy), ws)
    else:
        call('pidm_conv2d_wgrad_simt', x, dy, gw_buf, gb_buf, B, H, W, Cin, spec.cin_real, Ho, Wo, Cout, KH, KW,
             stride, pad, 1 if spec.transposed else 0, spec.w_stride_n, spec.w_stride_c, _code(x), ws)
    return dx, gw_ret, gb_ret


def conv2d(x, weight, bias, spec, residual=None, gn_link=None, skip=None):
    return _Conv2d.apply(x.contiguous(), weight, bias, None if residual is None else residual.contiguous(), spec,
                         gn_link, skip)


class _GroupNormSilu(torch.autograd.Function):
    @staticmethod
    def forward(ctx, x, gamma, beta, scale_shift, groups, eps, link, residual):
        B, H, W, C = x.shape
        y = torch.empty_like(x)
        pre = link is not None and link.get('sums') is not None
        sums = link['sums'] if pre else torch.empty(B, groups, 2, device=x.device, dtype=torch.float32)
        call('pidm_groupnorm_silu_fwd', x, gamma, beta, scale_shift, residual, y, sums, 1 if pre else 0, B, H * W, C,
             groups, eps, _code(x), stream())
        ctx.save_for_backward(x, gamma, beta, scale_shift, sums)
        ctx.groups, ctx.eps, ctx.link, ctx.has_res = groups, eps, link, residual is not None
        return y

    @staticmethod
    def backward(ctx, dy):
        x, gamma, beta, ss, sums = ctx.saved_tensors
        B, H, W, C = x.shape
        dy = dy.contiguous()
        dx = torch.empty_like(x)
        gg_buf, gg_ret = _grad_buffer(gamma)
        gb_buf, gb_ret = _grad_buffer(beta)
        dss = None if ss is None else torch.empty_like(ss)
        ws = torch.empty(B * C * 2, device=x.device, dtype=torch.float32)
        dbias = None
        link = ctx.link
        if link is not None and link.get('bias') is not None:
            dbias, dbias_ret = _grad_buffer(link['bias'])
            link['dbias'] = dbias_ret
        call('pidm_groupnorm_silu_bwd', x, dy, sums, gamma, beta, ss, dx, gg_buf, gb_buf, dss, dbias, ws, B, H * W, C,
             ctx.groups, ctx.eps, _code(x), stream())
        return dx, gg_ret, gb_ret, dss, None, None, None, (dy if ctx.has_res else None)


def groupnorm_silu(x, gamma, beta, scale_shift, groups, eps=1e-5, gn_link=None, residual=None):
    return _GroupNormSilu.apply(x.contiguous(), gamma, beta, scale_shift, groups, eps, gn_link,
                                None if residual is None else residual.contiguous())


class _LayerNormC(torch.autograd.Function):
    @staticmethod
    def forward(ctx, x, gamma, eps, skip_link):
        C = x.shape[-1]
        y = torch.empty_like(x)
        call('pidm_layernorm_c_fwd', x, gamma, y, x.numel() // C, C, eps, _code(x), stream())
        ctx.save_for_backward(x, gamma)
        ctx.eps, ctx.skip_link = eps, skip_link
        return y

    @staticmethod
    def backward(ctx, dy):
        x, gamma = ctx.saved_tensors
        C = x.shape[-1]
        dy = dy.contiguous()
        dx = torch.empty_like(x)
        gg_buf, gg_ret = _grad_buffer(gamma)
        call('pidm_layernorm_c_bwd', x, dy, gamma, dx, gg_buf,
             _take_skip(ctx.skip_link) if ctx.needs_input_grad[0] else None, x.numel() // C, C, ctx.eps,
             _code(x), stream())
        return dx, gg_ret, None, None


def layernorm_c(x, gamma, eps=1e-5, skip_link=None):
    return _LayerNormC.apply(x.contiguous(), gamma, eps, skip_link)


class _LinAttn(torch.autograd.Function):
    @staticmethod
    def forward(ctx, qkv, heads):
        B, H, W, C3 = qkv.shape
        N = H * W
        hid = heads * 32
        assert C3 == 3 * hid
        out = torch.empty(B, H, W, hid, device=qkv.device, dtype=qkv.dtype)
        ctxm = torch.empty(B, heads, 32, 32, device=qkv.device, dtype=torch.float32)
        kmax = torch.empty(B, heads, 32, device=qkv.device, dtype=torch.float32)
        kzinv = torch.empty_like(kmax)
        ws = torch.empty(call('pidm_linattn_workspace_floats', B, N, heads), device=qkv.device, dtype=torch.float32)
        call('pidm_linattn_fwd', qkv, out, ctxm, kmax, kzinv, ws, B, N, heads, _code(qkv), stream())
        ctx.save_for_backward(qkv, ctxm, kmax, kzinv)
        ctx.heads = heads
        return out

    @staticmethod
    def backward(ctx, dout):
        qkv, ctxm, kmax, kzinv = ctx.saved_tensors
        B, H, W, _ = qkv.shape
        dout = dout.contiguous()
        dqkv = torch.empty_like(qkv)
        dctx = torch.empty_like(ctxm)
        call('pidm_linattn_bwd', qkv, dout, ctxm, kmax, kzinv, dqkv, dctx, B, H * W, ctx.heads, _code(qkv), stream())
        return dqkv, None


class _LinAttnFused(torch.autograd.Function):

    @staticmethod
    def forward(ctx, xn, weight, spec, heads):
        B, H, W, C = xn.shape
        N = H * W
        out = torch.empty(B, H, W, heads * 32, device=xn.device, dtype=xn.dtype)
        ctxm = torch.empty(B, heads, 32, 32, device=xn.device, dtype=torch.float32)
        kmax = torch.empty(B, heads, 32, device=xn.device, dtype=torch.float32)
        kzinv = torch.empty_like(kmax)
        ws = torch.empty(call('pidm_linattn_fused_workspace_floats', B, N), device=xn.device, dtype=torch.float32)
        call('pidm_linattn_fused_fwd', xn, spec.wp_fwd, out, ctxm, kmax, kzinv, ws, B, N, stream())
        ctx.save_for_backward(xn, weight, ctxm, kmax, kzinv)
        ctx.spec, ctx.heads = spec, heads
        return out

    @staticmethod
    def backward(ctx, dout):
        xn, weight, ctxm, kmax, kzinv = ctx.saved_tensors
        spec = ctx.spec
        B, H, W, _ = xn.shape
        dout = dout.contiguous()
        dx = torch.empty_like(xn)
        dctx = torch.empty_like(ctxm)
        call('pidm_linattn_fused_bwd', xn, spec.wp_fwd, dout, ctxm, kmax, kzinv, dx, dctx, B, H * W, stream())
        gw_buf, gw_ret = _grad_buffer(weight)
        ws = _wgrad_stream(xn, spec.wp_fwd, dout, ctxm, dctx, kmax, kzinv)
        call('pidm_linattn_fused_wgrad', xn, spec.wp_fwd, dout, ctxm, dctx, kmax, kzinv, gw_buf, B, H * W,
             spec.w_stride_n, spec.w_stride_c, ws)
        return (dx if ctx.needs_input_grad[0] else None), gw_ret, None, None


def linear_attention_fused_supported(xn, spec, heads):
    B, H, W, C = xn.shape
    return (_STATE['use_tc'] and xn.is_cuda and spec.kh == 1 and spec.kw == 1 and spec.cout == 3 * heads * 32
            and bool(call('pidm_linattn_fused_supported', C, heads, H * W, _code(xn))))


def linear_attention_fused(xn, weight, spec, heads):
    return _LinAttnFused.apply(xn.contiguous(), weight, spec, heads)


def linear_attention(qkv, heads):
    return _LinAttn.apply(qkv.contiguous(), heads)


class _Attn(torch.autograd.Function):
    @staticmethod
    def forward(ctx, qkv, heads):
        B, H, W, C3 = qkv.shape
        out = torch.empty(B, H, W, heads * 32, device=qkv.device, dtype=qkv.dtype)
        call('pidm_attn_fwd', qkv, out, B, H * W, heads, _code(qkv), stream())
        ctx.save_for_backward(qkv)
        ctx.heads = heads
        return out

    @staticmethod
    def backward(ctx, dout):
        (qkv,) = ctx.saved_tensors
        B, H, W, _ = qkv.shape
        dqkv = torch.empty_like(qkv)
        call('pidm_attn_bwd', qkv, dout.contiguous(), dqkv, B, H * W, ctx.heads, _code(qkv), stream())
        return dqkv, None


def softmax_attention(qkv, heads):
    return _Attn.apply(qkv.contiguous(), heads)


class _TimeEmbed(torch.autograd.Function):
    @staticmethod
    def forward(ctx, t, W1, b1, W2, b2):
        B = t.shape[0]
        td, dim = W1.shape
        dev = W1.device
        emb = torch.empty(B, dim, device=dev, dtype=torch.float32)
        h1 = torch.empty(B, td, device=dev, dtype=torch.float32)
        temb = torch.empty_like(h1)
        silu_t = torch.empty_like(h1)
        call('pidm_time_embed_fwd', t, W1, b1, W2, b2, emb, h1, temb, silu_t, B, dim, td, stream())
        ctx.save_for_backward(emb, h1, temb, W1, b1, W2, b2)
        ctx.mark_non_differentiable(temb)
        return silu_t, temb

    @staticmethod
    def backward(ctx, d_silu, _unused):
        emb, h1, temb, W1, b1, W2, b2 = ctx.saved_tensors
        B, td = h1.shape
        gW1, rW1 = _grad_buffer(W1)
        gb1, rb1 = _grad_buffer(b1)
        gW2, rW2 = _grad_buffer(W2)
        gb2, rb2 = _grad_buffer(b2)
        d_silu = d_silu.contiguous()
        ws = torch.empty(2 * B * td, device=h1.device, dtype=torch.float32)
        args = (d_silu, emb, h1, temb, W2, gW1, gb1, gW2, gb2, ws, B, emb.shape[1], td)
        call('pidm_time_embed_bwd', *args, 2, stream())
        call('pidm_time_embed_bwd', *args, 1, _wgrad_stream(ws, emb, h1))
        return None, rW1, rb1, rW2, rb2


def time_embed(t, W1, b1, W2, b2):
    return _TimeEmbed.apply(t.to(torch.int64).contiguous(), W1, b1, W2, b2)


class _BlockMlps(torch.autograd.Function):

    @staticmethod
    def forward(ctx, silu_t, table, *wb):
        B, td = silu_t.shape
        outs = [torch.empty(B, n, device=silu_t.device, dtype=torch.float32) for n in table.rows]
        call('pidm_block_mlps_fwd', table.device_table(outs), table.n, table.max_rows, silu_t, B, td, stream())
        ctx.save_for_backward(silu_t, *wb)
        ctx.table = table
        return tuple(outs)

    @staticmethod
    def backward(ctx, *d_outs):
        silu_t, *wb = ctx.saved_tensors
        table = ctx.table
        B, td = silu_t.shape
        bufs, rets = [], []
        for p in wb:
            b_, r_ = _grad_buffer(p)
            bufs.append(b_)
            rets.append(r_)
        d_outs = [d.contiguous() for d in d_outs]
        d_silu = torch.empty_like(silu_t)
        tab = table.device_table(None, d_outs, bufs)
        call('pidm_block_mlps_bwd', tab, table.n, table.max_rows, silu_t, d_silu, B, td, 1,
             _wgrad_stream(silu_t, tab, *d_outs))
        call('pidm_block_mlps_bwd', tab, table.n, table.max_rows, silu_t, d_silu, B, td, 2, stream())
        return (d_silu, None, *rets)


def block_mlps(silu_t, table):
    return _BlockMlps.apply(silu_t, table, *table.params)


class _Head(torch.autograd.Function):
    @staticmethod
    def forward(ctx, x, w, b, sigmoid_last):
        B, H, W, C = x.shape
        O = w.shape[0]
        y = torch.empty(B, O, H, W, device=x.device, dtype=torch.float32)
        call('pidm_head_fwd', x, w, b, y, B, H * W, C, O, int(sigmoid_last), _code(x), stream())
        ctx.save_for_backward(x, w, b, y)
        ctx.sig = int(sigmoid_last)
        return y

    @staticmethod
    def backward(ctx, dy):
        x, w, b, y = ctx.saved_tensors
        B, H, W, C = x.shape
        O = w.shape[0]
        dx = torch.empty_like(x)
        gw, rw = _grad_buffer(w)
        gb, rb = _grad_buffer(b)
        call('pidm_head_bwd', x, w, y, dy.contiguous().float(), dx, gw, gb, B, H * W, C, O, ctx.sig, _code(x), stream())
        return dx, rw, rb, None


def head(x, w, b, sigmoid_last=False):
    return _Head.apply(x.contiguous(), w, b, sigmoid_last)


def q_sample(x0, noise, t, sqrt_ab, sqrt_1mab):
    _need_cuda(x0, noise, t)
    _need_f32(sqrt_ab=sqrt_ab, sqrt_1mab=sqrt_1mab)
    x0 = x0.contiguous().float()
    xt = torch.empty_like(x0)
    call('pidm_qsample', x0, noise.contiguous().float(), t.to(torch.int64).contiguous(), sqrt_ab, sqrt_1mab, xt,
         x0.shape[0], x0[0].numel(), stream())
    return xt


def posterior_step(x_t, x0_pred, z, c1, c2, sigma):
    out = torch.empty_like(x_t)
    call('pidm_posterior_step', x_t.contiguous(), x0_pred.contiguous(), z.contiguous(), out, float(c1), float(c2),
         float(sigma), x_t.numel(), stream())
    return out


class _DarcyResidual(torch.autograd.Function):
    @staticmethod
    def forward(ctx, x0hat, f_s, geom):
        B, C, P, _ = x0hat.shape
        r = torch.empty(B, P * P, 3, device=x0hat.device, dtype=torch.float32)
        call('pidm_darcy_residual_fwd', x0hat, f_s, r, B, P, *geom, stream())
        ctx.save_for_backward(x0hat, f_s)
        ctx.geom = geom
        return r

    @staticmethod
    def backward(ctx, gr):
        x0hat, f_s = ctx.saved_tensors
        B, C, P, _ = x0hat.shape
        gx = torch.empty_like(x0hat)
        call('pidm_darcy_residual_bwd', x0hat, f_s, gr.contiguous(), gx, B, P, *ctx.geom, stream())
        return gx, None, None


DARCY_PIXELS_AT_BOUNDARY = 1
DARCY_PERIODIC = 2


def darcy_flags(pixels_at_boundary, periodic=False):
    return (DARCY_PIXELS_AT_BOUNDARY if pixels_at_boundary else 0) | (DARCY_PERIODIC if periodic else 0)


def darcy_residual(x0hat, f_s, domain_length=1.0, reverse_d1=True, pixels_at_boundary=True, periodic=False):
    _need_cuda(x0hat)
    _need_f32(f_s=f_s)
    assert x0hat.shape[1] == 2, 'Darcy fields are (p, K)'
    return _DarcyResidual.apply(x0hat.contiguous().float(), f_s,
                                (float(domain_length), int(reverse_d1), darcy_flags(pixels_at_boundary, periodic)))


class _DarcyPidmLoss(torch.autograd.Function):

    @staticmethod
    def forward(ctx, x0hat, model_out, target, t, f_s, p2w, pvar, c_data, c_res, geom):
        B, C, P, _ = x0hat.shape
        same = model_out is None
        sums = torch.empty(3, device=x0hat.device, dtype=torch.float32)
        need = x0hat.requires_grad or (model_out is not None and model_out.requires_grad)
        gx = torch.empty_like(x0hat) if need else None
        gm = None if (same or not need) else torch.empty_like(model_out)
        call('pidm_darcy_pidm_loss', x0hat, x0hat if same else model_out, target, f_s, t, p2w, pvar, float(c_data),
             float(c_res), sums, gx, gm, B, P, *geom, stream())
        ctx.save_for_backward(gx, gm)
        ctx.mark_non_differentiable(sums)
        return sums[0] + sums[1], sums

    @staticmethod
    def backward(ctx, g, _unused):
        gx, gm = ctx.saved_tensors
        g = g.contiguous().float()
        ox = torch.empty_like(gx)
        call('pidm_scale', gx, g, ox, gx.numel(), stream())
        om = None
        if gm is not None:
            om = torch.empty_like(gm)
            call('pidm_scale', gm, g, om, gm.numel(), stream())
        return ox, om, None, None, None, None, None, None, None, None


def darcy_pidm_loss(x0hat, model_out, target, t, f_s, p2w, pvar, c_data, c_res, domain_length=1.0, reverse_d1=True,
                    pixels_at_boundary=True, periodic=False):
    _need_cuda(x0hat, target)
    _need_f32(f_s=f_s, p2w=p2w, pvar=pvar)
    geom = (float(domain_length), int(reverse_d1), darcy_flags(pixels_at_boundary, periodic))
    if model_out is not None and model_out is x0hat:
        model_out = None
    return _DarcyPidmLoss.apply(x0hat.contiguous().float(),
                                None if model_out is None else model_out.contiguous().float(),
                                target.contiguous().float(), t.to(torch.int64).contiguous(), f_s, p2w, pvar, c_data, c_res,
                                geom)
```

physicsinformeddiffusionmodels_b200/unet_model.py:

```python
import math

import torch
from torch import nn

from . import ops
from .packing import ConvSpec, MlpTable, WeightPacker


def exists(x):
    return x is not None


def default(val, d):
    if exists(val):
        return val
    return d() if callable(d) else d


def _round_up(x, m):
    return (x + m - 1) // m * m


class RotaryEmbedding(nn.Module):

    def __init__(self, dim, theta=10000):
        super().__init__()
        freqs = 1.0 / (theta ** (torch.arange(0, dim, 2)[: (dim // 2)].float() / dim))
        self.freqs = nn.Parameter(freqs, requires_grad=False)


class RelativePositionBias(nn.Module):
    def __init__(self, heads=8, num_buckets=32, max_distance=128):
        super().__init__()
        self.relative_attention_bias = nn.Embedding(num_buckets, heads)


class LayerNorm(nn.Module):
    def __init__(self, dim, eps=1e-5):
        super().__init__()
        self.eps = eps
        self.gamma = nn.Parameter(torch.ones(1, dim, 1, 1, 1))


class PreNorm(nn.Module):
    def __init__(self, dim, fn):
        super().__init__()
        self.fn = fn
        self.norm = LayerNorm(dim)


class Residual(nn.Module):
    def __init__(self, fn):
        super().__init__()
        self.fn = fn


class EinopsToAndFrom(nn.Module):
    def __init__(self, fn):
        super().__init__()
        self.fn = fn


class Attention(nn.Module):

    def __init__(self, dim, heads=4, dim_head=32, rotary_emb=None, cond_dim=64):
        super().__init__()
        self.heads, self.dim_head = heads, dim_head
        hidden = dim_head * heads
        self.rotary_emb = rotary_emb
        self.to_qkv = nn.Linear(dim, hidden * 3, bias=False)
        self.to_q = nn.Linear(dim, hidden, bias=False)
        self.to_k = nn.Linear(cond_dim, hidden, bias=False)
        self.to_v = nn.Linear(cond_dim, hidden, bias=False)
        self.to_out = nn.Conv2d(hidden, dim, 1)
        self.to_out = nn.Linear(hidden, dim, bias=False)


class SpatialLinearAttention(nn.Module):
    def __init__(self, dim, heads=4, dim_head=32, cond_dim=64):
        super().__init__()
        self.heads = heads
        hidden = dim_head * heads
        self.to_qkv = nn.Conv2d(dim, hidden * 3, 1, bias=False)
        self.to_q = nn.Conv2d(dim, hidden, 1, bias=False)
        self.to_k = nn.Linear(cond_dim, hidden, bias=False)
        self.to_v = nn.Linear(cond_dim, hidden, bias=False)
        self.to_out = nn.Conv2d(hidden, dim, 1)


class Block(nn.Module):
    def __init__(self, dim, dim_out, groups=8):
        super().__init__()
        self.proj = nn.Conv3d(dim, dim_out, (1, 3, 3), padding=(0, 1, 1))
        self.norm = nn.GroupNorm(groups, dim_out)


class ResnetBlock(nn.Module):
    def __init__(self, dim, dim_out, *, time_emb_dim=None, groups=8):
        super().__init__()
        self.mlp = nn.Sequential(nn.SiLU(), nn.Linear(time_emb_dim, dim_out * 2)) if exists(time_emb_dim) else None
        self.block1 = Block(dim, dim_out, groups=groups)
        self.block2 = Block(dim_out, dim_out, groups=groups)
        self.res_conv = nn.Conv3d(dim, dim_out, 1) if dim != dim_out else nn.Identity()
        self.groups = groups


class SignalEmbedding(nn.Module):

    def __init__(self, init_channel, channel_upsamplings):
        super().__init__()
        scale = [init_channel, *channel_upsamplings]
        mods = []
        for ci, co in zip(scale[:-1], scale[1:]):
            mods += [nn.Conv1d(ci, co, kernel_size=4, stride=2, padding=1), nn.SiLU()]
        self.emb_model = nn.Sequential(*mods)


class Unet3D(nn.Module):
    def __init__(self, dim, out_dim=None, dim_mults=(1, 2, 4, 8), channels=2, self_condition=False, attn_heads=8,
                 attn_dim_head=32, init_dim=None, init_kernel_size=7, use_sparse_linear_attn=True, resnet_groups=8,
                 cond_bias=False, cond_attention='none', cond_attention_tokens=6, cond_to_time='add',
                 padding_mode='zeros', sigmoid_last_channel=False):
        super().__init__()
        if padding_mode != 'zeros':
            raise NotImplementedError("only padding_mode='zeros' (the reference default) is implemented")
        if not use_sparse_linear_attn:
            raise NotImplementedError('use_sparse_linear_attn=False is not used by the reference drivers')
        if attn_dim_head != 32:
            raise NotImplementedError('attention kernels are built for dim_head = 32 (reference default)')
        if self_condition:
            raise NotImplementedError('self_condition=True is not used by the reference drivers')
        assert init_kernel_size % 2 == 1
        self.input_channels = channels
        self.self_condition = self_condition
        self.dim = dim
        time_dim = dim * 4
        self.cond_dim = time_dim
        self.cond_to_time = cond_to_time
        self.padding_mode = padding_mode
        self.heads = attn_heads
        self.groups = resnet_groups
        self.init_kernel_size = init_kernel_size

        rotary_emb = RotaryEmbedding(min(32, attn_dim_head))

        def temporal_attn(d):
            return EinopsToAndFrom(Attention(d, heads=attn_heads, dim_head=attn_dim_head, rotary_emb=rotary_emb,
                                             cond_dim=self.cond_dim))
        self.time_rel_pos_bias = RelativePositionBias(heads=attn_heads, max_distance=32)
        init_dim = default(init_dim, dim)
        pad = init_kernel_size // 2
        self.init_conv = nn.Conv3d(channels, init_dim, (1, init_kernel_size, init_kernel_size), padding=(0, pad, pad))
        self.init_temporal_attn = Residual(PreNorm(init_dim, temporal_attn(init_dim)))
        dims = [init_dim, *map(lambda m: dim * m, dim_mults)]
        in_out = list(zip(dims[:-1], dims[1:]))
        self.time_mlp = nn.Sequential(nn.Identity(), nn.Linear(dim, time_dim), nn.GELU(), nn.Linear(time_dim, time_dim))
        self.sign_emb_CNN = SignalEmbedding(1, (16, 32, 64, 128, self.cond_dim))
        self.downs = nn.ModuleList([])
        self.ups = nn.ModuleList([])
        n_res = len(in_out)
        tdim = time_dim + int(self.cond_dim or 0) if cond_to_time == 'concat' else self.cond_dim

        def rb(a, b, time=True):
            return ResnetBlock(a, b, time_emb_dim=tdim if time else None, groups=resnet_groups)

        def lin_attn(d):
            return Residual(PreNorm(d, SpatialLinearAttention(d, heads=attn_heads, cond_dim=self.cond_dim)))
        for ind, (di, do) in enumerate(in_out):
            is_last = ind >= (n_res - 1)
            self.downs.append(nn.ModuleList([
                rb(di, do), rb(do, do), lin_attn(do),
                nn.Conv3d(do, do, (1, 4, 4), (1, 2, 2), (0, 1, 1)) if not is_last else nn.Identity()]))
        mid = dims[-1]
        self.mid_block1 = rb(mid, mid)
        spatial_attn = EinopsToAndFrom(Attention(mid, heads=attn_heads, cond_dim=self.cond_dim))
        self.mid_spatial_attn = Residual(PreNorm(mid, spatial_attn))
        self.mid_temporal_attn = Residual(PreNorm(mid, temporal_attn(mid)))
        self.mid_block2 = rb(mid, mid)
        for ind, (di, do) in enumerate(reversed(in_out)):
            is_last = ind >= (n_res - 1)
            self.ups.append(nn.ModuleList([
                rb(do * 2, di), rb(di, di), lin_attn(di),
                nn.ConvTranspose3d(di, di, (1, 4, 4), (1, 2, 2), (0, 1, 1)) if not is_last else nn.Identity()]))
        out_dim = default(out_dim, channels)
        self.out_dim = out_dim
        self.final_conv = nn.Sequential(rb(dim * 2, dim, time=False), nn.Conv3d(dim, out_dim, 1))
        self.emb_conv = nn.Sequential(nn.Conv2d(channels, init_dim, kernel_size=1), nn.GELU(),
                                      nn.Conv2d(init_dim, init_dim, kernel_size=3, padding=1))
        self.combine_conv = nn.Conv2d(init_dim * 2, init_dim, kernel_size=1)
        self.sigmoid_last_channel = sigmoid_last_channel

        self._build_plan()

    def _build_plan(self):
        pk = WeightPacker()
        self._packer = pk
        self._cin_pad = _round_up(self.input_channels, 32)
        k = self.init_kernel_size
        self._spec = {}

        def conv(mod, kh, stride, pad, kind='conv', cin_pad=None, need_dgrad=True):
            s = pk.add(ConvSpec(mod.weight, kind, kh, kh, stride, pad, cin_pad=cin_pad, need_dgrad=need_dgrad))
            self._spec[id(mod)] = s
            return s
        conv(self.init_conv, k, 1, k // 2, cin_pad=self._cin_pad, need_dgrad=False)
        mlps = []

        def plan_rb(block):
            conv(block.block1.proj, 3, 1, 1)
            conv(block.block2.proj, 3, 1, 1)
            if not isinstance(block.res_conv, nn.Identity):
                conv(block.res_conv, 1, 1, 0)
            if block.mlp is not None:
                block._mlp_index = len(mlps)
                mlps.append(block.mlp[1])

        def plan_la(res):
            conv(res.fn.fn.to_qkv, 1, 1, 0)
            conv(res.fn.fn.to_out, 1, 1, 0)
        self._early_specs = 0
        for b1, b2, la, down in self.downs:
            plan_rb(b1); plan_rb(b2); plan_la(la)
            if self._early_specs == 0:
                self._early_specs = len(pk.specs)
            if not isinstance(down, nn.Identity):
                conv(down, 4, 2, 1)
        plan_rb(self.mid_block1)
        att = self.mid_spatial_attn.fn.fn.fn
        conv(att.to_qkv, 1, 1, 0)
        conv(att.to_out, 1, 1, 0)
        plan_rb(self.mid_block2)
        for b1, b2, la, up in self.ups:
            plan_rb(b1); plan_rb(b2); plan_la(la)
            if not isinstance(up, nn.Identity):
                conv(up, 4, 2, 1, kind='convT')
        plan_rb(self.final_conv[0])
        conv(self.emb_conv[0], 1, 1, 0, cin_pad=self._cin_pad, need_dgrad=False)
        conv(self.emb_conv[2], 3, 1, 1)
        conv(self.combine_conv, 1, 1, 0)
        self._mlp_table = MlpTable(mlps)

    def unused_parameter_names(self):
        dead = []
        for name, p in self.named_parameters():
            if not p.requires_grad:
                continue
            parts = name.split('.')
            if (name.startswith(('time_rel_pos_bias.', 'sign_emb_CNN.', 'emb_conv.', 'combine_conv.', 'init_temporal_attn.',
                                 'mid_temporal_attn.'))
                    or parts[-2] in ('to_q', 'to_k', 'to_v')):
                dead.append(name)
        return dead

    _boundary_cb = None

    def _boundary(self, group, h):
        cb = self._boundary_cb
        if cb is not None and h.requires_grad:
            h.register_hook(lambda g, _cb=cb, _k=group: _cb(_k))
        return h

    def _conv(self, mod, x, residual=None, gn_link=None, skip=None):
        return ops.conv2d(x, mod.weight, getattr(mod, 'bias', None), self._spec[id(mod)], residual=residual,
                          gn_link=gn_link, skip=skip)

    def _resblock(self, block, x, ss_list):
        ss = ss_list[block._mlp_index] if (block.mlp is not None and ss_list is not None) else None
        l1, l2 = {'groups': block.groups}, {'groups': block.groups}
        sk = {}
        h = self._conv(block.block1.proj, x, gn_link=l1, skip=('take', sk))
        h = ops.groupnorm_silu(h, block.block1.norm.weight, block.block1.norm.bias, ss, block.groups,
                               block.block1.norm.eps, gn_link=l1)
        h = self._conv(block.block2.proj, h, gn_link=l2)
        if isinstance(block.res_conv, nn.Identity):
            return ops.groupnorm_silu(h, block.block2.norm.weight, block.block2.norm.bias, None, block.groups,
                                      block.block2.norm.eps, gn_link=l2, residual=ops.stash_grad(x, sk))
        h = ops.groupnorm_silu(h, block.block2.norm.weight, block.block2.norm.bias, None, block.groups,
                               block.block2.norm.eps, gn_link=l2)
        return self._conv(block.res_conv, x, residual=h, skip=('park', sk))

    def _linear_attention(self, res, x):
        pre = res.fn
        sk = {}
        xn = ops.layernorm_c(x, pre.norm.gamma, pre.norm.eps, skip_link=sk)
        to_qkv = pre.fn.to_qkv
        spec = self._spec[id(to_qkv)]
        if getattr(to_qkv, 'bias', None) is None and ops.linear_attention_fused_supported(xn, spec, pre.fn.heads):
            a = ops.linear_attention_fused(xn, to_qkv.weight, spec, pre.fn.heads)
        else:
            qkv = self._conv(to_qkv, xn)
            a = ops.linear_attention(qkv, pre.fn.heads)
        return self._conv(pre.fn.to_out, a, residual=ops.stash_grad(x, sk))

    def _mid_attention(self, res, x):
        pre = res.fn
        att = pre.fn.fn
        sk = {}
        xn = ops.layernorm_c(x, pre.norm.gamma, pre.norm.eps, skip_link=sk)
        qkv = self._conv(att.to_qkv, xn)
        a = ops.softmax_attention(qkv, att.heads)
        return self._conv(att.to_out, a, residual=ops.stash_grad(x, sk))

    def forward_with_guidance_scale(self, *args, **kwargs):
        from .denoising_utils import _axpby
        guidance_scale = kwargs.pop('guidance_scale', 3.)
        logits = self.forward(*args, null_cond_prob=0., **kwargs)
        if guidance_scale == 1:
            return logits
        null_logits = self.forward(*args, null_cond_prob=1., **kwargs)
        B = logits.shape[0]
        full = lambda v: torch.full((B,), float(v), device=logits.device, dtype=torch.float32)
        return _axpby(full(guidance_scale), logits, full(1. - guidance_scale), null_logits, full(0.), null_logits)

    def _cond_embedding(self, h, cond, null_cond_prob):
        from .denoising_utils import _axpby
        if cond.dim() != 3:
            raise ValueError('Input must be [BxP*PxC].')
        B, N, C = cond.shape
        P = int(math.isqrt(N))
        mask = getattr(self, '_null_mask_override', None)
        if mask is None:
            if null_cond_prob == 1:
                mask = torch.ones(B, device=cond.device, dtype=torch.bool)
            elif null_cond_prob == 0:
                mask = torch.zeros(B, device=cond.device, dtype=torch.bool)
            else:
                mask = torch.zeros(B, device=cond.device).float().uniform_(0, 1) < null_cond_prob
        cimg = cond.detach().reshape(B, P, P, C).permute(0, 3, 1, 2).contiguous().float()
        keep = (~mask).float().contiguous()
        zero = torch.zeros_like(keep)
        cimg = _axpby(keep, cimg, zero, cimg, zero, cimg)
        e = ops.nchw_to_nhwc(cimg, self._cin_pad, ops.act_dtype())
        e = self._conv(self.emb_conv[0], e)
        e = ops.gelu(e)
        e = self._conv(self.emb_conv[2], e)
        return self._conv(self.combine_conv, ops.concat(h, e))

    def forward(self, x, time, x_self_cond=None, cond=None, null_cond_prob=0.):
        if exists(x_self_cond):
            raise NotImplementedError('self-conditioning is not used by the reference drivers')
        video = False
        if x.dim() == 3:
            B, N, C = x.shape
            P = int(math.isqrt(N))
            assert P * P == N, 'number of pixels must be a perfect square'
            x = x.reshape(B, P, P, C).permute(0, 3, 1, 2)
        elif x.dim() == 5:
            if x.shape[2] != 1:
                raise NotImplementedError('image sequences with F > 1 frames are not used by the reference drivers')
            x = x[:, :, 0]
            video = True
        elif x.dim() != 4:
            raise ValueError('Input must be image [BxCxPxP] or image sequence [BxCxFxPxP].')
        if not x.is_cuda:
            raise RuntimeError('Unet3D (CUDA engine) needs CUDA tensors: no CPU fallback on the product path')
        dt = ops.act_dtype()
        pack_stream = ops.fork_stream()
        early_packed = None
        if torch.is_grad_enabled() or self._packer.stale(dt):
            with torch.cuda.stream(pack_stream):
                early_packed = self._packer.refresh(dt, early_specs=0 if exists(cond) else self._early_specs)
        ops.zero_pool_begin(64 * (x.shape[0] * self.groups * 2 + 32), x.device)
        h = ops.nchw_to_nhwc(x.float(), self._cin_pad, dt)
        tm = self.time_mlp
        if time.dim() == 0:
            time = time.reshape(1).expand(x.shape[0])
        silu_t, _ = ops.time_embed(time, tm[1].weight, tm[1].bias, tm[3].weight, tm[3].bias)
        ss = ops.block_mlps(silu_t, self._mlp_table)
        if early_packed is not None:
            torch.cuda.current_stream().wait_event(early_packed)
        else:
            torch.cuda.current_stream().wait_stream(pack_stream)
        h = self._conv(self.init_conv, h)
        if exists(cond):
            h = self._cond_embedding(h, cond, null_cond_prob)
        r = h
        skips = []
        for lvl, (b1, b2, la, down) in enumerate(self.downs):
            if lvl == 2:
                h = self._boundary(1, h)
            h = self._resblock(b1, h, ss)
            h = self._resblock(b2, h, ss)
            h = self._linear_attention(la, h)
            skips.append(h)
            if lvl == 0 and early_packed is not None:
                torch.cuda.current_stream().wait_stream(pack_stream)
            if not isinstance(down, nn.Identity):
                h = self._conv(down, h)
        h = self._resblock(self.mid_block1, h, ss)
        h = self._mid_attention(self.mid_spatial_attn, h)
        h = self._resblock(self.mid_block2, h, ss)
        h = self._boundary(2, h)
        for b1, b2, la, up in self.ups:
            h = ops.concat(h, skips.pop())
            h = self._resblock(b1, h, ss)
            h = self._resblock(b2, h, ss)
            h = self._linear_attention(la, h)
            if not isinstance(up, nn.Identity):
                h = self._conv(up, h)
        h = ops.concat(h, r)
        h = self._resblock(self.final_conv[0], h, None)
        fc = self.final_conv[1]
        y = ops.head(h, fc.weight, fc.bias, self.sigmoid_last_channel)
        ops.zero_pool_end()
        return y.unsqueeze(2) if video else y
```

Before: 6573.

## Fuse linear-attention output projection, bias and residual into fused attention kernels

Extends the fused linear-attention forward, backward and weight-gradient kernels with a PROJ variant. The variant applies the to_out 1x1 projection, bias and residual add inside the kernel and folds the projection's input gradient into the dcontext and backward passes. This removes the separate to_out convolution launches and the round trip of the hidden-width attention output through global memory. In exchange it adds shared-memory usage, block-wide syncs and a cross-warp reduction through shared memory in the output kernel.

```diff
diff --git a/include/pidm.h b/include/pidm.h
--- a/include/pidm.h
+++ b/include/pidm.h
@@ -102,6 +102,14 @@
 int pidm_linattn_fused_wgrad(const void* xn, const void* w_qkv, const void* dout, const float* ctx, const float* dctx,
                              const float* kmax, const float* kzinv, float* grad_w, int B, int N, long long w_stride_n,
                              long long w_stride_c, void* stream);
+int pidm_linattn_block_fwd(const void* xn, const void* w_qkv, const void* w_out, const float* b_out, const void* residual,
+                           void* y, float* ctx, float* kmax, float* kzinv, float* workspace, int B, int N, void* stream);
+int pidm_linattn_block_bwd(const void* xn, const void* w_qkv, const void* w_out, const void* dy, const float* ctx,
+                           const float* kmax, const float* kzinv, void* dxn, float* dctx, int B, int N, void* stream);
+int pidm_linattn_block_wgrad(const void* xn, const void* w_qkv, const void* w_out, const void* dy, const float* ctx,
+                             const float* dctx, const float* kmax, const float* kzinv, float* grad_w_qkv,
+                             long long qkv_stride_n, long long qkv_stride_c, float* grad_w_out, long long out_stride_n,
+                             long long out_stride_c, int B, int N, void* stream);
 int pidm_linattn_workspace_floats(int B, int N, int heads);
 int pidm_linattn_fwd(const void* qkv, void* out, float* ctx, float* kmax, float* kzinv, float* workspace, int B, int N,
                      int heads, int dtype, void* stream);
diff --git a/physicsinformeddiffusionmodels_b200/_lib.py b/physicsinformeddiffusionmodels_b200/_lib.py
--- a/physicsinformeddiffusionmodels_b200/_lib.py
+++ b/physicsinformeddiffusionmodels_b200/_lib.py
@@ -56,6 +56,9 @@
     'pidm_linattn_fused_fwd': [P, P, P, P, P, P, P, I, I, P],
     'pidm_linattn_fused_bwd': [P, P, P, P, P, P, P, P, I, I, P],
     'pidm_linattn_fused_wgrad': [P, P, P, P, P, P, P, P, I, I, L, L, P],
+    'pidm_linattn_block_fwd': [P, P, P, P, P, P, P, P, P, P, I, I, P],
+    'pidm_linattn_block_bwd': [P, P, P, P, P, P, P, P, P, I, I, P],
+    'pidm_linattn_block_wgrad': [P, P, P, P, P, P, P, P, P, L, L, P, L, L, I, I, P],
     'pidm_linattn_fwd': [P, P, P, P, P, P, I, I, I, I, P],
     'pidm_linattn_bwd': [P, P, P, P, P, P, P, I, I, I, I, P],
     'pidm_attn_fwd': [P, P, I, I, I, I, P],
diff --git a/physicsinformeddiffusionmodels_b200/csrc/attention_fused.cu b/physicsinformeddiffusionmodels_b200/csrc/attention_fused.cu
--- a/physicsinformeddiffusionmodels_b200/csrc/attention_fused.cu
+++ b/physicsinformeddiffusionmodels_b200/csrc/attention_fused.cu
@@ -143,17 +143,46 @@
     if (lane == 0) kzinv[row] = zi;
 }
 
-template <int MODE>
+constexpr int LFP_WO_TILE = LF_C * LW_PITCH;
+
+__device__ __forceinline__ void lfp_dout_acc(float (&c)[4][4], const uint32_t (&ady)[2][4], const __nv_bfloat16* Wo, int lane) {
+#pragma unroll
+    for (int nt = 0; nt < 4; ++nt)
+#pragma unroll
+        for (int i = 0; i < 4; ++i) c[nt][i] = 0.f;
+#pragma unroll
+    for (int kc = 0; kc < 2; ++kc)
+#pragma unroll
+        for (int np = 0; np < 2; ++np) {
+            uint32_t bw[4];
+            frag_b_krows(bw, Wo, LW_PITCH, kc * 16, np * 16, lane);
+            mma_bf16(c[2 * np], ady[kc], bw[0], bw[1]);
+            mma_bf16(c[2 * np + 1], ady[kc], bw[2], bw[3]);
+        }
+}
+__device__ __forceinline__ void lfp_dout(uint32_t (&ag)[2][4], const __nv_bfloat16* dyt, const __nv_bfloat16* Wo, int lane) {
+    uint32_t ady[2][4];
+    frag_a_rowmajor(ady[0], dyt, LW_PITCH, 0, 0, lane);
+    frag_a_rowmajor(ady[1], dyt, LW_PITCH, 0, 16, lane);
+    float c[4][4];
+    lfp_dout_acc(c, ady, Wo, lane);
+    c_to_a(ag, c);
+}
+
+template <int MODE, bool PROJ = false>
 struct LfcCfg {
     static constexpr int STAGES = MODE == 0 ? 4 : 2;
     static constexpr int STAGE_ELEMS = MODE == 0 ? LW_TILE : 2 * LW_TILE;
-    static constexpr size_t SMEM = (size_t)LM_HEADS * STAGES * STAGE_ELEMS * 2 + (size_t)LM_HEADS * 2 * LM_D * 4;
+    static constexpr size_t SMEM = (size_t)LM_HEADS * STAGES * STAGE_ELEMS * 2 + (size_t)LM_HEADS * 2 * LM_D * 4 +
+                                   (PROJ ? (size_t)LM_HEADS * LFP_WO_TILE * 2 : 0);
 };
-template <int MODE>
+template <int MODE, bool PROJ = false>
 __global__ void __launch_bounds__(256, 2) laf_ctx_kernel(const __nv_bfloat16* __restrict__ xn, const __nv_bfloat16* __restrict__ W,
                                                       const __nv_bfloat16* __restrict__ dout, const float* __restrict__ part,
                                                       int n_stat_chunks, float* __restrict__ kmax, float* __restrict__ kzinv,
-                                                      float* __restrict__ ctx, int N, int chunk_px, float scale) {
+                                                      float* __restrict__ ctx, int N, int chunk_px, float scale,
+                                                      const __nv_bfloat16* __restrict__ w_out) {
+    static_assert(!PROJ || MODE == 1, "PROJ applies to the dcontext pass");
     pdl_trigger();
     pdl_wait();
     extern __shared__ __align__(16) unsigned char raw[];
@@ -162,16 +191,22 @@
     __nv_bfloat16* ring = reinterpret_cast<__nv_bfloat16*>(raw) + (size_t)h * (LFC_STAGES * LFC_STAGE_ELEMS);
     float* sM = reinterpret_cast<float*>(raw + (size_t)LM_HEADS * LFC_STAGES * LFC_STAGE_ELEMS * 2) + h * 2 * LM_D;
     float* sZi = sM + LM_D;
+    __nv_bfloat16* Wo = reinterpret_cast<__nv_bfloat16*>(raw + LfcCfg<MODE>::SMEM) + h * LFP_WO_TILE;
     const int n_begin = chunk * chunk_px, n_end = min(N, n_begin + chunk_px);
     const int n_tiles = (n_end - n_begin) / 32;
     const size_t pix0 = (size_t)b * N + n_begin;
     const __nv_bfloat16* xsrc = xn + pix0 * LF_C;
-    const __nv_bfloat16* gsrc = (MODE == 1) ? dout + pix0 * LM_HID + h * LM_D : nullptr;
+    const __nv_bfloat16* gsrc = (MODE == 1) ? (PROJ ? dout + pix0 * LF_C : dout + pix0 * LM_HID + h * LM_D) : nullptr;
+    constexpr int G_STRIDE = PROJ ? LF_C : LM_HID;
+    if (PROJ) {
+        lw_issue<32>(Wo, w_out + h * LM_D, LM_HID, lane);
+        cp_commit();
+    }
     auto issue = [&](int it) {
         if (it < n_tiles) {
             __nv_bfloat16* buf = ring + (size_t)(it % LFC_STAGES) * LFC_STAGE_ELEMS;
             lw_issue<32>(buf, xsrc + (size_t)it * 32 * LF_C, LF_C, lane);
-            if (MODE == 1) lw_issue<32>(buf + LW_TILE, gsrc + (size_t)it * 32 * LM_HID, LM_HID, lane);
+            if (MODE == 1) lw_issue<32>(buf + LW_TILE, gsrc + (size_t)it * 32 * G_STRIDE, G_STRIDE, lane);
         }
         cp_commit();
     };
@@ -207,7 +242,21 @@
         uint32_t ax[2][2][4];
         load_x_frags<2>(ax, buf, lane);
         uint32_t bv[2][4][2];
-        if (MODE == 1) {
+        if (PROJ) {
+#pragma unroll
+            for (int mt = 0; mt < 2; ++mt) {
+                uint32_t ady[2][4];
+                frag_a_rowmajor(ady[0], buf + LW_TILE, LW_PITCH, mt * 16, 0, lane);
+                frag_a_rowmajor(ady[1], buf + LW_TILE, LW_PITCH, mt * 16, 16, lane);
+                float cd[4][4];
+                lfp_dout_acc(cd, ady, Wo, lane);
+#pragma unroll
+                for (int nt = 0; nt < 4; ++nt) {
+                    bv[mt][nt][0] = movm_t(pack_bf16(cd[nt][0], cd[nt][1]));
+                    bv[mt][nt][1] = movm_t(pack_bf16(cd[nt][2], cd[nt][3]));
+                }
+            }
+        } else if (MODE == 1) {
 #pragma unroll
             for (int ks = 0; ks < 2; ++ks) {
                 uint32_t b01[4], b23[4];
@@ -289,26 +338,42 @@
 }
 
 constexpr int LFO_STAGES = 2;
+constexpr int LFOP_STAGES = 3;
+constexpr int LFO_R_PITCH = LF_C + 8;
+constexpr size_t LAF_OUT_PROJ_SMEM = (size_t)LFOP_STAGES * LW_TILE * 2 + (size_t)LM_HEADS * LFP_WO_TILE * 2 +
+                                     (size_t)LM_HEADS * 32 * LFO_R_PITCH * 4;
+template <bool PROJ = false>
 __global__ void __launch_bounds__(256) laf_out_kernel(const __nv_bfloat16* __restrict__ xn, const __nv_bfloat16* __restrict__ W,
                                                       const float* __restrict__ ctx, __nv_bfloat16* __restrict__ out, int N,
-                                                      int chunk_px, float scale) {
+                                                      int chunk_px, float scale, const __nv_bfloat16* __restrict__ w_out,
+                                                      const float* __restrict__ b_out,
+                                                      const __nv_bfloat16* __restrict__ residual) {
     pdl_trigger();
     pdl_wait();
     extern __shared__ __align__(16) unsigned char raw[];
+    constexpr int STAGES = PROJ ? LFOP_STAGES : LFO_STAGES;
     const int b = blockIdx.y, chunk = blockIdx.x, lane = threadIdx.x & 31, h = threadIdx.x >> 5;
-    __nv_bfloat16* ring = reinterpret_cast<__nv_bfloat16*>(raw) + (size_t)h * ((LFO_STAGES + 1) * LW_TILE);
+    __nv_bfloat16* ring = reinterpret_cast<__nv_bfloat16*>(raw) + (PROJ ? 0 : (size_t)h * ((LFO_STAGES + 1) * LW_TILE));
     __nv_bfloat16* Os = ring + LFO_STAGES * LW_TILE;
+    __nv_bfloat16* Wo = reinterpret_cast<__nv_bfloat16*>(raw) + LFOP_STAGES * LW_TILE + h * LFP_WO_TILE;
+    float* R = reinterpret_cast<float*>(reinterpret_cast<__nv_bfloat16*>(raw) + LFOP_STAGES * LW_TILE +
+                                        LM_HEADS * LFP_WO_TILE);
     const int n_begin = chunk * chunk_px, n_end = min(N, n_begin + chunk_px);
     const int n_tiles = (n_end - n_begin) / 32;
     const size_t pix0 = (size_t)b * N + n_begin;
     const __nv_bfloat16* xsrc = xn + pix0 * LF_C;
     __nv_bfloat16* odst = out + pix0 * LM_HID + h * LM_D;
+    if (PROJ) {
+        lw_issue<32>(Wo, w_out + h * LM_D, LM_HID, lane);
+        cp_commit();
+    }
     auto issue = [&](int it) {
-        if (it < n_tiles) lw_issue<32>(ring + (size_t)(it % LFO_STAGES) * LW_TILE, xsrc + (size_t)it * 32 * LF_C, LF_C, lane);
+        if (it < n_tiles && (!PROJ || h == 0))
+            lw_issue<32>(ring + (size_t)(it % STAGES) * LW_TILE, xsrc + (size_t)it * 32 * LF_C, LF_C, lane);
         cp_commit();
     };
 #pragma unroll
-    for (int s = 0; s < LFO_STAGES; ++s) issue(s);
+    for (int s = 0; s < (PROJ ? STAGES - 1 : STAGES); ++s) issue(s);
     uint32_t wq[2][4][2];
     load_w_frags(wq, W + (size_t)(h * LM_D) * LF_C, lane);
     const float* ch = ctx + ((size_t)b * LM_HEADS + h) * LM_D * LM_D;
@@ -318,13 +383,29 @@
 #pragma unroll
         for (int nt = 0; nt < 4; ++nt) frag_b_global<true>(bf[ks][nt], ch, ks * 16, nt * 8, lane);
     const int g = lane >> 2, t = lane & 3;
+    const int rrow = threadIdx.x >> 4, rcol = (threadIdx.x & 15) * 2;
+    float2 bias = make_float2(0.f, 0.f);
+    if (PROJ) bias = make_float2(b_out[rcol], b_out[rcol + 1]);
+    float* Rw = R + h * 32 * LFO_R_PITCH;
     for (int it = 0; it < n_tiles; ++it) {
-        cp_wait<LFO_STAGES - 1>();
-        __syncwarp();
         uint32_t ax[2][2][4];
-        load_x_frags<2>(ax, ring + (size_t)(it % LFO_STAGES) * LW_TILE, lane);
-        __syncwarp();
-        issue(it + LFO_STAGES);
+        if (PROJ) {
+            cp_wait<STAGES - 2>();
+            __syncthreads();
+            issue(it + STAGES - 1);
+            load_x_frags<2>(ax, ring + (size_t)(it % STAGES) * LW_TILE, lane);
+        } else {
+            cp_wait<LFO_STAGES - 1>();
+            __syncwarp();
+            load_x_frags<2>(ax, ring + (size_t)(it % LFO_STAGES) * LW_TILE, lane);
+            __syncwarp();
+            issue(it + LFO_STAGES);
+        }
+        __nv_bfloat162 res[2];
+        if (PROJ)
+#pragma unroll
+            for (int rh = 0; rh < 2; ++rh)
+                res[rh] = *reinterpret_cast<const __nv_bfloat162*>(residual + (pix0 + (size_t)it * 32 + rrow + rh * 16) * LF_C + rcol);
         float cq[2][4][4];
         project<2>(cq, ax, wq);
 #pragma unroll
@@ -341,16 +422,58 @@
             for (int ks = 0; ks < 2; ++ks)
 #pragma unroll
                 for (int nt = 0; nt < 4; ++nt) mma_bf16(c[nt], a[ks], bf[ks][nt][0], bf[ks][nt][1]);
-#pragma unroll
-            for (int nt = 0; nt < 4; ++nt) {
-                __nv_bfloat16* o = Os + (size_t)(mt * 16 + g) * LW_PITCH + nt * 8 + 2 * t;
-                *reinterpret_cast<uint32_t*>(o) = pack_bf16(c[nt][0], c[nt][1]);
-                *reinterpret_cast<uint32_t*>(o + 8 * LW_PITCH) = pack_bf16(c[nt][2], c[nt][3]);
+            if (PROJ) {
+                c_to_a(a, c);
+                float y[4][4];
+#pragma unroll
+                for (int i = 0; i < 4; ++i)
+#pragma unroll
+                    for (int k = 0; k < 4; ++k) y[i][k] = 0.f;
+#pragma unroll
+                for (int ke = 0; ke < 2; ++ke)
+#pragma unroll
+                    for (int np = 0; np < 2; ++np) {
+                        uint32_t bw[4];
+                        frag_b_nrows(bw, Wo, LW_PITCH, np * 16, ke * 16, lane);
+                        mma_bf16(y[2 * np], a[ke], bw[0], bw[1]);
+                        mma_bf16(y[2 * np + 1], a[ke], bw[2], bw[3]);
+                    }
+#pragma unroll
+                for (int nt = 0; nt < 4; ++nt)
+#pragma unroll
+                    for (int half = 0; half < 2; ++half)
+                        *reinterpret_cast<float2*>(Rw + (mt * 16 + g + half * 8) * LFO_R_PITCH + nt * 8 + 2 * t) =
+                            make_float2(y[nt][half * 2], y[nt][half * 2 + 1]);
+            } else {
+#pragma unroll
+                for (int nt = 0; nt < 4; ++nt) {
+                    __nv_bfloat16* o = Os + (size_t)(mt * 16 + g) * LW_PITCH + nt * 8 + 2 * t;
+                    *reinterpret_cast<uint32_t*>(o) = pack_bf16(c[nt][0], c[nt][1]);
+                    *reinterpret_cast<uint32_t*>(o + 8 * LW_PITCH) = pack_bf16(c[nt][2], c[nt][3]);
+                }
             }
         }
-        __syncwarp();
-        lw_store<32>(odst + (size_t)it * 32 * LM_HID, LM_HID, Os, lane);
-        __syncwarp();
+        if (PROJ) {
+            __syncthreads();
+#pragma unroll
+            for (int rh = 0; rh < 2; ++rh) {
+                const int row = rrow + rh * 16;
+                const size_t pix = pix0 + (size_t)it * 32 + row;
+                const float2 x = __bfloat1622float2(res[rh]);
+                float sx = x.x + bias.x, sy = x.y + bias.y;
+#pragma unroll
+                for (int w = 0; w < LM_HEADS; ++w) {
+                    const float2 v = *reinterpret_cast<const float2*>(R + (w * 32 + row) * LFO_R_PITCH + rcol);
+                    sx += v.x;
+                    sy += v.y;
+                }
+                *reinterpret_cast<uint32_t*>(out + pix * LF_C + rcol) = pack_bf16(sx, sy);
+            }
+        } else {
+            __syncwarp();
+            lw_store<32>(odst + (size_t)it * 32 * LM_HID, LM_HID, Os, lane);
+            __syncwarp();
+        }
     }
 }
 
@@ -435,11 +558,15 @@
     load_cols(cdc, scd, lane);
 }
 
-constexpr int LFB_STAGE_ELEMS = (1 + LM_HEADS) * LFB_TILE;
 constexpr int LFB_W_PITCH = LF_C + 8;
 constexpr int LFB_R_PITCH = LF_C + 8;
-constexpr size_t LAF_BWD_SMEM = (size_t)LFB_STAGES * LFB_STAGE_ELEMS * 2 + (size_t)3 * LM_HID * LFB_W_PITCH * 2 +
-                                (size_t)LM_HEADS * LFB_ROWS * LFB_R_PITCH * 4 + (size_t)LM_HEADS * LM_D * 4;
+template <bool PROJ>
+struct LfbCfg {
+    static constexpr int STAGE_ELEMS = (PROJ ? 2 : 1 + LM_HEADS) * LFB_TILE;
+    static constexpr size_t SMEM_BASE = (size_t)LFB_STAGES * STAGE_ELEMS * 2 + (size_t)3 * LM_HID * LFB_W_PITCH * 2 +
+                                        (size_t)LM_HEADS * LFB_ROWS * LFB_R_PITCH * 4 + (size_t)LM_HEADS * LM_D * 4;
+    static constexpr size_t SMEM = SMEM_BASE + (PROJ ? (size_t)LM_HEADS * LFP_WO_TILE * 2 : 0);
+};
 
 __device__ __forceinline__ void mma_w(float (&c)[4][4], const uint32_t (&g)[2][4], const __nv_bfloat16* Wh, int lane) {
 #pragma unroll
@@ -453,32 +580,37 @@
         }
 }
 
+template <bool PROJ = false>
 __global__ void __launch_bounds__(256) laf_bwd_kernel(const __nv_bfloat16* __restrict__ xn, const __nv_bfloat16* __restrict__ W,
                                                       const __nv_bfloat16* __restrict__ dout, const float* __restrict__ ctx,
                                                       const float* __restrict__ dctx, const float* __restrict__ kmax,
                                                       const float* __restrict__ kzinv, __nv_bfloat16* __restrict__ dxn,
-                                                      int N, int chunk_px, float scale) {
+                                                      int N, int chunk_px, float scale, const __nv_bfloat16* __restrict__ w_out) {
     pdl_trigger();
     pdl_wait();
     extern __shared__ __align__(16) unsigned char raw[];
+    constexpr int LFB_STAGE_ELEMS = LfbCfg<PROJ>::STAGE_ELEMS;
     const int b = blockIdx.y, chunk = blockIdx.x, lane = threadIdx.x & 31, h = threadIdx.x >> 5;
     __nv_bfloat16* ring = reinterpret_cast<__nv_bfloat16*>(raw);
     __nv_bfloat16* Ws = ring + LFB_STAGES * LFB_STAGE_ELEMS;
+    __nv_bfloat16* Wo = reinterpret_cast<__nv_bfloat16*>(raw + LfbCfg<PROJ>::SMEM_BASE) + h * LFP_WO_TILE;
     float* R = reinterpret_cast<float*>(Ws + 3 * LM_HID * LFB_W_PITCH);
     float* scd = R + LM_HEADS * LFB_ROWS * LFB_R_PITCH + h * LM_D;
     const int n_begin = chunk * chunk_px, n_end = min(N, n_begin + chunk_px);
     const int n_tiles = (n_end - n_begin) / LFB_ROWS;
     const size_t pix0 = (size_t)b * N + n_begin;
     const __nv_bfloat16* xsrc = xn + pix0 * LF_C;
-    const __nv_bfloat16* gsrc = dout + pix0 * LM_HID + h * LM_D;
+    const __nv_bfloat16* gsrc = PROJ ? dout + pix0 * LF_C : dout + pix0 * LM_HID + h * LM_D;
     for (int i = threadIdx.x; i < 3 * LM_HID * (LF_C / 8); i += blockDim.x)
         cp_async16(Ws + (i >> 2) * LFB_W_PITCH + (i & 3) * 8, W + (size_t)(i >> 2) * LF_C + (i & 3) * 8);
+    if (PROJ) lw_issue<32>(Wo, w_out + h * LM_D, LM_HID, lane);
     cp_commit();
     auto issue = [&](int it) {
         if (it < n_tiles) {
             __nv_bfloat16* buf = ring + (size_t)(it % LFB_STAGES) * LFB_STAGE_ELEMS;
             if (h == 0) lw_issue<LFB_ROWS>(buf, xsrc + (size_t)it * LFB_ROWS * LF_C, LF_C, lane);
-            lw_issue<LFB_ROWS>(buf + (1 + h) * LFB_TILE, gsrc + (size_t)it * LFB_ROWS * LM_HID, LM_HID, lane);
+            if (!PROJ) lw_issue<LFB_ROWS>(buf + (1 + h) * LFB_TILE, gsrc + (size_t)it * LFB_ROWS * LM_HID, LM_HID, lane);
+            else if (h == 1) lw_issue<LFB_ROWS>(buf + LFB_TILE, gsrc + (size_t)it * LFB_ROWS * LF_C, LF_C, lane);
         }
         cp_commit();
     };
@@ -517,8 +649,12 @@
         const __nv_bfloat16* buf = ring + (size_t)(it % LFB_STAGES) * LFB_STAGE_ELEMS;
         LfbTile tl;
         load_x_frags<1>(tl.ax, buf, lane);
-        frag_a_rowmajor(tl.ag[0], buf + (1 + h) * LFB_TILE, LW_PITCH, 0, 0, lane);
-        frag_a_rowmajor(tl.ag[1], buf + (1 + h) * LFB_TILE, LW_PITCH, 0, 16, lane);
+        if (PROJ) {
+            lfp_dout(tl.ag, buf + LFB_TILE, Wo, lane);
+        } else {
+            frag_a_rowmajor(tl.ag[0], buf + (1 + h) * LFB_TILE, LW_PITCH, 0, 0, lane);
+            frag_a_rowmajor(tl.ag[1], buf + (1 + h) * LFB_TILE, LW_PITCH, 0, 16, lane);
+        }
         float dx[4][4];
 #pragma unroll
         for (int nt = 0; nt < 4; ++nt)
@@ -557,13 +693,15 @@
     }
 }
 
-template <int PART>
+template <int PART, bool PROJ = false>
 struct LfwCfg {
-    static constexpr int MATS = PART == 0 ? 1 : 2;
+    static_assert(!PROJ || PART == 0, "PROJ applies to part 0");
+    static constexpr int MATS = (PART == 0 && !PROJ) ? 1 : 2;
     static constexpr int STAGE_ELEMS = (PART == 0 ? 2 : 1) * LFB_TILE;
     static constexpr int S_PITCH = LM_D + 1;
     static_assert(LFB_STAGES * STAGE_ELEMS * 2 >= LM_D * S_PITCH * 4, "the epilogue staging reuses the tile ring");
-    static constexpr size_t SMEM = (size_t)LM_HEADS * (LFB_STAGES * STAGE_ELEMS * 2 + LM_D * 4);
+    static constexpr size_t SMEM_BASE = (size_t)LM_HEADS * (LFB_STAGES * STAGE_ELEMS * 2 + LM_D * 4);
+    static constexpr size_t SMEM = SMEM_BASE + (PROJ ? (size_t)LM_HEADS * LFP_WO_TILE * 2 : 0);
 };
 
 __device__ __forceinline__ void acc_gtx(float (&acc)[2][4][4], const float (&gf)[4][4], const uint32_t (&bx)[2][4]) {
@@ -582,29 +720,38 @@
     }
 }
 
-template <int PART>
+template <int PART, bool PROJ = false>
 __global__ void __launch_bounds__(256) laf_wgrad_kernel(const __nv_bfloat16* __restrict__ xn, const __nv_bfloat16* __restrict__ W,
                                                         const __nv_bfloat16* __restrict__ dout, const float* __restrict__ ctx,
                                                         const float* __restrict__ dctx, const float* __restrict__ kmax,
                                                         const float* __restrict__ kzinv, float* __restrict__ grad_w, int N,
-                                                        int chunk_px, long long w_stride_n, long long w_stride_c, float scale) {
+                                                        int chunk_px, long long w_stride_n, long long w_stride_c, float scale,
+                                                        const __nv_bfloat16* __restrict__ w_out, float* __restrict__ grad_wo,
+                                                        long long wo_stride_n, long long wo_stride_c) {
     pdl_trigger();
     pdl_wait();
     extern __shared__ __align__(16) unsigned char raw[];
-    constexpr int MATS = LfwCfg<PART>::MATS, STAGE_ELEMS = LfwCfg<PART>::STAGE_ELEMS, S_PITCH = LfwCfg<PART>::S_PITCH;
+    using Cfg = LfwCfg<PART, PROJ>;
+    constexpr int MATS = Cfg::MATS, STAGE_ELEMS = Cfg::STAGE_ELEMS, S_PITCH = Cfg::S_PITCH;
     const int b = blockIdx.y, chunk = blockIdx.x, lane = threadIdx.x & 31, h = threadIdx.x >> 5;
     __nv_bfloat16* ring = reinterpret_cast<__nv_bfloat16*>(raw) + (size_t)h * (LFB_STAGES * STAGE_ELEMS);
     float* scd = reinterpret_cast<float*>(raw + (size_t)LM_HEADS * LFB_STAGES * STAGE_ELEMS * 2) + h * LM_D;
+    __nv_bfloat16* Wo = reinterpret_cast<__nv_bfloat16*>(raw + Cfg::SMEM_BASE) + h * LFP_WO_TILE;
     const int n_begin = chunk * chunk_px, n_end = min(N, n_begin + chunk_px);
     const int n_tiles = (n_end - n_begin) / LFB_ROWS;
     const size_t pix0 = (size_t)b * N + n_begin;
     const __nv_bfloat16* xsrc = xn + pix0 * LF_C;
-    const __nv_bfloat16* gsrc = dout + pix0 * LM_HID + h * LM_D;
+    const __nv_bfloat16* gsrc = PROJ ? dout + pix0 * LF_C : dout + pix0 * LM_HID + h * LM_D;
+    constexpr int G_STRIDE = PROJ ? LF_C : LM_HID;
+    if (PROJ) {
+        lw_issue<32>(Wo, w_out + h * LM_D, LM_HID, lane);
+        cp_commit();
+    }
     auto issue = [&](int it) {
         if (it < n_tiles) {
             __nv_bfloat16* buf = ring + (size_t)(it % LFB_STAGES) * STAGE_ELEMS;
             lw_issue<LFB_ROWS>(buf, xsrc + (size_t)it * LFB_ROWS * LF_C, LF_C, lane);
-            if (PART == 0) lw_issue<LFB_ROWS>(buf + LFB_TILE, gsrc + (size_t)it * LFB_ROWS * LM_HID, LM_HID, lane);
+            if (PART == 0) lw_issue<LFB_ROWS>(buf + LFB_TILE, gsrc + (size_t)it * LFB_ROWS * G_STRIDE, G_STRIDE, lane);
         }
         cp_commit();
     };
@@ -629,7 +776,7 @@
 #pragma unroll
         for (int nt = 0; nt < 4; ++nt) {
             frag_b_global<false>(b0[ks][nt], PART == 0 ? cg : dg, ks * 16, nt * 8, lane);
-            if (PART == 1) frag_b_global<true>(b1[ks][nt], dg, ks * 16, nt * 8, lane);
+            if (PART == 1 || PROJ) frag_b_global<true>(b1[ks][nt], PART == 1 ? dg : cg, ks * 16, nt * 8, lane);
         }
     const float invN = 1.f / (float)N;
     float acc[MATS][2][4][4];
@@ -650,16 +797,42 @@
         uint32_t bx[2][4];
         frag_b_krows(bx[0], buf, LW_PITCH, 0, 0, lane);
         frag_b_krows(bx[1], buf, LW_PITCH, 0, 16, lane);
-        if (PART == 0) {
+        uint32_t ady[2][4], bdy[2][4];
+        if (PROJ) {
+            frag_a_rowmajor(ady[0], buf + LFB_TILE, LW_PITCH, 0, 0, lane);
+            frag_a_rowmajor(ady[1], buf + LFB_TILE, LW_PITCH, 0, 16, lane);
+            frag_b_krows(bdy[0], buf + LFB_TILE, LW_PITCH, 0, 0, lane);
+            frag_b_krows(bdy[1], buf + LFB_TILE, LW_PITCH, 0, 16, lane);
+        } else if (PART == 0) {
             frag_a_rowmajor(tl.ag[0], buf + LFB_TILE, LW_PITCH, 0, 0, lane);
             frag_a_rowmajor(tl.ag[1], buf + LFB_TILE, LW_PITCH, 0, 16, lane);
         }
         __syncwarp();
         issue(it + LFB_STAGES);
         if (PART == 0) {
+            if (PROJ) {
+                float c[4][4];
+                lfp_dout_acc(c, ady, Wo, lane);
+                c_to_a(tl.ag, c);
+            }
             float dq[4][4];
             lfb_dq(dq, tl, w0, b0, scale);
             acc_gtx(acc[0], dq, bx);
+            if (PROJ) {
+                float cq[1][4][4], o[4][4];
+                project<1>(cq, tl.ax, w0);
+                frag_softmax(cq[0], scale);
+                uint32_t a[2][4];
+                c_to_a(a, cq[0]);
+#pragma unroll
+                for (int nt = 0; nt < 4; ++nt) {
+#pragma unroll
+                    for (int i = 0; i < 4; ++i) o[nt][i] = 0.f;
+#pragma unroll
+                    for (int ks = 0; ks < 2; ++ks) mma_bf16(o[nt], a[ks], b1[ks][nt][0], b1[ks][nt][1]);
+                }
+                acc_gtx(acc[MATS - 1], o, bdy);
+            }
         } else {
             float dk[4][4], dv[4][4];
             lfb_dkdv(dk, dv, tl.ax, w0, w1, b0, b1, Mc, Zc, cdc, invN);
@@ -680,9 +853,15 @@
 #pragma unroll
                 for (int i = 0; i < 4; ++i) S[(md * 16 + g + 8 * (i >> 1)) * S_PITCH + nc * 8 + 2 * t + (i & 1)] = acc[m][md][nc][i];
         __syncwarp();
-        float* dst = grad_w + (long long)((PART + m) * LM_HID + h * LM_D) * w_stride_n + lane * w_stride_c;
+        if (PROJ && m == 1) {
+            float* dst = grad_wo + (long long)(h * LM_D + lane) * wo_stride_c;
 #pragma unroll 4
-        for (int d = 0; d < LM_D; ++d) atomicAdd(dst + d * w_stride_n, S[d * S_PITCH + lane]);
+            for (int c = 0; c < LF_C; ++c) atomicAdd(dst + c * wo_stride_n, S[lane * S_PITCH + c]);
+        } else {
+            float* dst = grad_w + (long long)((PART + m) * LM_HID + h * LM_D) * w_stride_n + lane * w_stride_c;
+#pragma unroll 4
+            for (int d = 0; d < LM_D; ++d) atomicAdd(dst + d * w_stride_n, S[d * S_PITCH + lane]);
+        }
         __syncwarp();
     }
 }
@@ -696,9 +875,13 @@
         PIDM_CUDA(cudaFuncSetAttribute(laf_kmax_kernel, cudaFuncAttributeMaxDynamicSharedMemorySize, (int)LAF_STATS_SMEM));
         PIDM_CUDA(cudaFuncSetAttribute(laf_ctx_kernel<0>, cudaFuncAttributeMaxDynamicSharedMemorySize, (int)LfcCfg<0>::SMEM));
         PIDM_CUDA(cudaFuncSetAttribute(laf_ctx_kernel<1>, cudaFuncAttributeMaxDynamicSharedMemorySize, (int)LfcCfg<1>::SMEM));
-        PIDM_CUDA(cudaFuncSetAttribute(laf_out_kernel, cudaFuncAttributeMaxDynamicSharedMemorySize, (int)LAF_OUT_SMEM));
-        PIDM_CUDA(cudaFuncSetAttribute(laf_bwd_kernel, cudaFuncAttributeMaxDynamicSharedMemorySize, (int)LAF_BWD_SMEM));
+        PIDM_CUDA(cudaFuncSetAttribute(laf_ctx_kernel<1, true>, cudaFuncAttributeMaxDynamicSharedMemorySize, (int)LfcCfg<1, true>::SMEM));
+        PIDM_CUDA(cudaFuncSetAttribute(laf_out_kernel<false>, cudaFuncAttributeMaxDynamicSharedMemorySize, (int)LAF_OUT_SMEM));
+        PIDM_CUDA(cudaFuncSetAttribute(laf_out_kernel<true>, cudaFuncAttributeMaxDynamicSharedMemorySize, (int)LAF_OUT_PROJ_SMEM));
+        PIDM_CUDA(cudaFuncSetAttribute(laf_bwd_kernel<false>, cudaFuncAttributeMaxDynamicSharedMemorySize, (int)LfbCfg<false>::SMEM));
+        PIDM_CUDA(cudaFuncSetAttribute(laf_bwd_kernel<true>, cudaFuncAttributeMaxDynamicSharedMemorySize, (int)LfbCfg<true>::SMEM));
         PIDM_CUDA(cudaFuncSetAttribute(laf_wgrad_kernel<0>, cudaFuncAttributeMaxDynamicSharedMemorySize, (int)LfwCfg<0>::SMEM));
+        PIDM_CUDA(cudaFuncSetAttribute(laf_wgrad_kernel<0, true>, cudaFuncAttributeMaxDynamicSharedMemorySize, (int)LfwCfg<0, true>::SMEM));
         PIDM_CUDA(cudaFuncSetAttribute(laf_wgrad_kernel<1>, cudaFuncAttributeMaxDynamicSharedMemorySize, (int)LfwCfg<1>::SMEM));
         done = true;
     }
@@ -720,25 +903,9 @@
     return c;
 }
 
-}
-using namespace pidm;
-
-extern "C" int pidm_linattn_fused_supported(int C, int heads, int N, int dtype) {
-    return (C == LF_C && heads == LM_HEADS && dtype == PIDM_BF16 && N % 128 == 0) ? 1 : 0;
-}
-
-extern "C" int pidm_linattn_fused_workspace_floats(int B, int N) { return B * laf_stat_chunks(N) * LM_HID; }
-
-extern "C" int pidm_linattn_fused_plan(int B, int N, int* out) {
-    PIDM_REQUIRE(N % 128 == 0 && B > 0, "linattn_fused_plan: N must be a multiple of 128 (got %d)", N);
-    const int v[5] = {laf_stat_chunks(N), laf_chunk_px(B, N, 2), laf_chunk_px(B, N, 3), laf_chunk_px(B, N, 1),
-                      laf_chunk_px(B, N, 1)};
-    for (int i = 0; i < 5; ++i) out[i] = v[i];
-    return 0;
-}
-
-extern "C" int pidm_linattn_fused_fwd(const void* xn, const void* w_qkv, void* out, float* ctx, float* kmax, float* kzinv,
-                                      float* workspace, int B, int N, void* stream) {
+template <bool PROJ>
+static int laf_fwd(const void* xn, const void* w_qkv, const void* w_out, const float* b_out, const void* residual, void* out,
+                   float* ctx, float* kmax, float* kzinv, float* workspace, int B, int N, void* stream) {
     PIDM_REQUIRE(N % 128 == 0, "linattn_fused: N must be a multiple of 128 (got %d)", N);
     cudaStream_t st = (cudaStream_t)stream;
     if (int e = laf_attrs()) return e;
@@ -753,50 +920,113 @@
     PIDM_CUDA(launch_pdl(laf_kmax_kernel, dim3(dim3(chunks, B)), dim3(256), (size_t)(LAF_STATS_SMEM), st, x, w, workspace, N, rpc));
     const int cpx = laf_chunk_px(B, N, 2);
     PIDM_CUDA(launch_pdl(laf_ctx_kernel<0>, dim3(dim3((N + cpx - 1) / cpx, B)), dim3(256), (size_t)(LfcCfg<0>::SMEM), st, x, w, nullptr, workspace, chunks, kmax, kzinv,
-                                                                             ctx, N, cpx, scale));
+                                                                             ctx, N, cpx, scale, nullptr));
     PIDM_CUDA(launch_pdl(laf_finalize_kernel, dim3((B * LM_HID + 7) / 8), dim3(256), (size_t)(0), st, ctx, kzinv, B * LM_HID));
-    const int opx = laf_chunk_px(B, N, 3);
-    PIDM_CUDA(launch_pdl(laf_out_kernel, dim3(dim3((N + opx - 1) / opx, B)), dim3(256), (size_t)(LAF_OUT_SMEM), st, x, w, ctx, (__nv_bfloat16*)out, N, opx, scale));
+    const int opx = laf_chunk_px(B, N, PROJ ? 2 : 3);
+    PIDM_CUDA(launch_pdl(laf_out_kernel<PROJ>, dim3(dim3((N + opx - 1) / opx, B)), dim3(256),
+                         PROJ ? LAF_OUT_PROJ_SMEM : LAF_OUT_SMEM, st, x, w, ctx, (__nv_bfloat16*)out, N, opx, scale,
+                         (const __nv_bfloat16*)w_out, b_out, (const __nv_bfloat16*)residual));
     PIDM_LAUNCH_CHECK("linattn_fused_fwd");
     return 0;
 }
 
-extern "C" int pidm_linattn_fused_bwd(const void* xn, const void* w_qkv, const void* dout, const float* ctx,
-                                      const float* kmax, const float* kzinv, void* dxn, float* dctx, int B, int N,
-                                      void* stream) {
+template <bool PROJ>
+static int laf_bwd(const void* xn, const void* w_qkv, const void* w_out, const void* dout, const float* ctx,
+                   const float* kmax, const float* kzinv, void* dxn, float* dctx, int B, int N, void* stream) {
     PIDM_REQUIRE(N % 128 == 0, "linattn_fused: N must be a multiple of 128 (got %d)", N);
     cudaStream_t st = (cudaStream_t)stream;
     if (int e = laf_attrs()) return e;
     const float scale = 0.17677669529663687f;
     const __nv_bfloat16* x = (const __nv_bfloat16*)xn;
     const __nv_bfloat16* w = (const __nv_bfloat16*)w_qkv;
+    const __nv_bfloat16* wo = (const __nv_bfloat16*)w_out;
     PIDM_CUDA(cudaMemsetAsync(dctx, 0, (size_t)B * LM_HEADS * LM_D * LM_D * sizeof(float), st));
     const int cpx = laf_chunk_px(B, N, 2);
-    PIDM_CUDA(launch_pdl(laf_ctx_kernel<1>, dim3(dim3((N + cpx - 1) / cpx, B)), dim3(256), (size_t)(LfcCfg<1>::SMEM), st, x, w, (const __nv_bfloat16*)dout, nullptr, 0,
-                                                                             nullptr, nullptr, dctx, N, cpx, scale));
+    PIDM_CUDA(launch_pdl(laf_ctx_kernel<1, PROJ>, dim3(dim3((N + cpx - 1) / cpx, B)), dim3(256), LfcCfg<1, PROJ>::SMEM, st, x, w,
+                         (const __nv_bfloat16*)dout, nullptr, 0, nullptr, nullptr, dctx, N, cpx, scale, wo));
     const int bpx = laf_chunk_px(B, N, 1);
-    PIDM_CUDA(launch_pdl(laf_bwd_kernel, dim3(dim3((N + bpx - 1) / bpx, B)), dim3(256), (size_t)(LAF_BWD_SMEM), st, x, w, (const __nv_bfloat16*)dout, ctx, dctx, kmax,
-                                                                          kzinv, (__nv_bfloat16*)dxn, N, bpx, scale));
+    PIDM_CUDA(launch_pdl(laf_bwd_kernel<PROJ>, dim3(dim3((N + bpx - 1) / bpx, B)), dim3(256), LfbCfg<PROJ>::SMEM, st, x, w,
+                         (const __nv_bfloat16*)dout, ctx, dctx, kmax, kzinv, (__nv_bfloat16*)dxn, N, bpx, scale, wo));
     PIDM_LAUNCH_CHECK("linattn_fused_bwd");
     return 0;
 }
 
-extern "C" int pidm_linattn_fused_wgrad(const void* xn, const void* w_qkv, const void* dout, const float* ctx,
-                                        const float* dctx, const float* kmax, const float* kzinv, float* grad_w, int B,
-                                        int N, long long w_stride_n, long long w_stride_c, void* stream) {
+template <bool PROJ>
+static int laf_wgrad(const void* xn, const void* w_qkv, const void* w_out, const void* dout, const float* ctx,
+                     const float* dctx, const float* kmax, const float* kzinv, float* grad_w, long long w_stride_n,
+                     long long w_stride_c, float* grad_wo, long long wo_stride_n, long long wo_stride_c, int B, int N,
+                     void* stream) {
     PIDM_REQUIRE(N % 128 == 0, "linattn_fused: N must be a multiple of 128 (got %d)", N);
     cudaStream_t st = (cudaStream_t)stream;
     if (int e = laf_attrs()) return e;
     const float scale = 0.17677669529663687f;
     const __nv_bfloat16* x = (const __nv_bfloat16*)xn;
     const __nv_bfloat16* w = (const __nv_bfloat16*)w_qkv;
+    const __nv_bfloat16* wo = (const __nv_bfloat16*)w_out;
     const __nv_bfloat16* g = (const __nv_bfloat16*)dout;
     const int px = laf_chunk_px(B, N, 1);
     const dim3 grid((N + px - 1) / px, B);
-    PIDM_CUDA(launch_pdl(laf_wgrad_kernel<0>, grid, dim3(256), LfwCfg<0>::SMEM, st, x, w, g, ctx, dctx, kmax, kzinv, grad_w, N,
-                         px, w_stride_n, w_stride_c, scale));
+    PIDM_CUDA(launch_pdl(laf_wgrad_kernel<0, PROJ>, grid, dim3(256), LfwCfg<0, PROJ>::SMEM, st, x, w, g, ctx, dctx, kmax, kzinv,
+                         grad_w, N, px, w_stride_n, w_stride_c, scale, wo, grad_wo, wo_stride_n, wo_stride_c));
     PIDM_CUDA(launch_pdl(laf_wgrad_kernel<1>, grid, dim3(256), LfwCfg<1>::SMEM, st, x, w, g, ctx, dctx, kmax, kzinv, grad_w, N,
-                         px, w_stride_n, w_stride_c, scale));
+                         px, w_stride_n, w_stride_c, scale, nullptr, nullptr, 0LL, 0LL));
     PIDM_LAUNCH_CHECK("linattn_fused_wgrad");
     return 0;
 }
+
+}
+using namespace pidm;
+
+extern "C" int pidm_linattn_fused_supported(int C, int heads, int N, int dtype) {
+    return (C == LF_C && heads == LM_HEADS && dtype == PIDM_BF16 && N % 128 == 0) ? 1 : 0;
+}
+
+extern "C" int pidm_linattn_fused_workspace_floats(int B, int N) { return B * laf_stat_chunks(N) * LM_HID; }
+
+extern "C" int pidm_linattn_fused_plan(int B, int N, int* out) {
+    PIDM_REQUIRE(N % 128 == 0 && B > 0, "linattn_fused_plan: N must be a multiple of 128 (got %d)", N);
+    const int v[5] = {laf_stat_chunks(N), laf_chunk_px(B, N, 2), laf_chunk_px(B, N, 3), laf_chunk_px(B, N, 1),
+                      laf_chunk_px(B, N, 1)};
+    for (int i = 0; i < 5; ++i) out[i] = v[i];
+    return 0;
+}
+
+extern "C" int pidm_linattn_fused_fwd(const void* xn, const void* w_qkv, void* out, float* ctx, float* kmax, float* kzinv,
+                                      float* workspace, int B, int N, void* stream) {
+    return laf_fwd<false>(xn, w_qkv, nullptr, nullptr, nullptr, out, ctx, kmax, kzinv, workspace, B, N, stream);
+}
+
+extern "C" int pidm_linattn_fused_bwd(const void* xn, const void* w_qkv, const void* dout, const float* ctx,
+                                      const float* kmax, const float* kzinv, void* dxn, float* dctx, int B, int N,
+                                      void* stream) {
+    return laf_bwd<false>(xn, w_qkv, nullptr, dout, ctx, kmax, kzinv, dxn, dctx, B, N, stream);
+}
+
+extern "C" int pidm_linattn_fused_wgrad(const void* xn, const void* w_qkv, const void* dout, const float* ctx,
+                                        const float* dctx, const float* kmax, const float* kzinv, float* grad_w, int B,
+                                        int N, long long w_stride_n, long long w_stride_c, void* stream) {
+    return laf_wgrad<false>(xn, w_qkv, nullptr, dout, ctx, dctx, kmax, kzinv, grad_w, w_stride_n, w_stride_c, nullptr, 0, 0,
+                            B, N, stream);
+}
+
+extern "C" int pidm_linattn_block_fwd(const void* xn, const void* w_qkv, const void* w_out, const float* b_out,
+                                      const void* residual, void* y, float* ctx, float* kmax, float* kzinv,
+                                      float* workspace, int B, int N, void* stream) {
+    PIDM_REQUIRE(w_out && b_out && residual, "linattn_block_fwd: w_out, b_out and residual are required");
+    return laf_fwd<true>(xn, w_qkv, w_out, b_out, residual, y, ctx, kmax, kzinv, workspace, B, N, stream);
+}
+
+extern "C" int pidm_linattn_block_bwd(const void* xn, const void* w_qkv, const void* w_out, const void* dy, const float* ctx,
+                                      const float* kmax, const float* kzinv, void* dxn, float* dctx, int B, int N,
+                                      void* stream) {
+    return laf_bwd<true>(xn, w_qkv, w_out, dy, ctx, kmax, kzinv, dxn, dctx, B, N, stream);
+}
+
+extern "C" int pidm_linattn_block_wgrad(const void* xn, const void* w_qkv, const void* w_out, const void* dy,
+                                        const float* ctx, const float* dctx, const float* kmax, const float* kzinv,
+                                        float* grad_w_qkv, long long qkv_stride_n, long long qkv_stride_c,
+                                        float* grad_w_out, long long out_stride_n, long long out_stride_c, int B, int N,
+                                        void* stream) {
+    return laf_wgrad<true>(xn, w_qkv, w_out, dy, ctx, dctx, kmax, kzinv, grad_w_qkv, qkv_stride_n, qkv_stride_c,
+                           grad_w_out, out_stride_n, out_stride_c, B, N, stream);
+}
diff --git a/physicsinformeddiffusionmodels_b200/ops.py b/physicsinformeddiffusionmodels_b200/ops.py
--- a/physicsinformeddiffusionmodels_b200/ops.py
+++ b/physicsinformeddiffusionmodels_b200/ops.py
@@ -438,6 +438,53 @@
         return (dx if ctx.needs_input_grad[0] else None), gw_ret, None, None
 
 
+class _LinAttnBlock(torch.autograd.Function):
+
+    @staticmethod
+    def forward(ctx, xn, w_qkv, spec_qkv, w_out, b_out, spec_out, residual, heads):
+        B, H, W, C = xn.shape
+        N = H * W
+        y = torch.empty_like(residual)
+        ctxm = torch.empty(B, heads, 32, 32, device=xn.device, dtype=torch.float32)
+        kmax = torch.empty(B, heads, 32, device=xn.device, dtype=torch.float32)
+        kzinv = torch.empty_like(kmax)
+        ws = torch.empty(call('pidm_linattn_fused_workspace_floats', B, N), device=xn.device, dtype=torch.float32)
+        call('pidm_linattn_block_fwd', xn, spec_qkv.wp_fwd, spec_out.wp_fwd, b_out, residual, y, ctxm, kmax, kzinv, ws,
+             B, N, stream())
+        ctx.save_for_backward(xn, w_qkv, w_out, b_out, ctxm, kmax, kzinv)
+        ctx.specs = (spec_qkv, spec_out)
+        return y
+
+    @staticmethod
+    def backward(ctx, dy):
+        xn, w_qkv, w_out, b_out, ctxm, kmax, kzinv = ctx.saved_tensors
+        sq, so = ctx.specs
+        B, H, W, _ = xn.shape
+        N = H * W
+        dy = dy.contiguous()
+        dx = torch.empty_like(xn)
+        dctx = torch.empty_like(ctxm)
+        call('pidm_linattn_block_bwd', xn, sq.wp_fwd, so.wp_fwd, dy, ctxm, kmax, kzinv, dx, dctx, B, N, stream())
+        gq_buf, gq_ret = _grad_buffer(w_qkv)
+        go_buf, go_ret = _grad_buffer(w_out)
+        gb_buf, gb_ret = _grad_buffer(b_out)
+        ws = _wgrad_stream(xn, sq.wp_fwd, so.wp_fwd, dy, ctxm, dctx, kmax, kzinv)
+        call('pidm_linattn_block_wgrad', xn, sq.wp_fwd, so.wp_fwd, dy, ctxm, dctx, kmax, kzinv, gq_buf, sq.w_stride_n,
+             sq.w_stride_c, go_buf, so.w_stride_n, so.w_stride_c, B, N, ws)
+        call('pidm_colsum', dy, gb_buf, B * N, dy.shape[-1], _code(dy), ws)
+        return (dx if ctx.needs_input_grad[0] else None), gq_ret, None, go_ret, gb_ret, None, dy, None
+
+
+def linear_attention_block_supported(xn, spec_qkv, spec_out, b_out, heads):
+    return (b_out is not None and spec_out.kh == 1 and spec_out.kw == 1 and not spec_out.transposed
+            and spec_out.cin == heads * 32 and spec_out.cout == xn.shape[-1]
+            and linear_attention_fused_supported(xn, spec_qkv, heads))
+
+
+def linear_attention_block(xn, w_qkv, spec_qkv, w_out, b_out, spec_out, residual, heads):
+    return _LinAttnBlock.apply(xn.contiguous(), w_qkv, spec_qkv, w_out, b_out, spec_out, residual.contiguous(), heads)
+
+
 def linear_attention_fused_supported(xn, spec, heads):
     B, H, W, C = xn.shape
     return (_STATE['use_tc'] and xn.is_cuda and spec.kh == 1 and spec.kw == 1 and spec.cout == 3 * heads * 32
diff --git a/physicsinformeddiffusionmodels_b200/unet_model.py b/physicsinformeddiffusionmodels_b200/unet_model.py
--- a/physicsinformeddiffusionmodels_b200/unet_model.py
+++ b/physicsinformeddiffusionmodels_b200/unet_model.py
@@ -285,6 +285,12 @@
         xn = ops.layernorm_c(x, pre.norm.gamma, pre.norm.eps, skip_link=sk)
         to_qkv = pre.fn.to_qkv
         spec = self._spec[id(to_qkv)]
+        to_out = pre.fn.to_out
+        b_out = getattr(to_out, 'bias', None)
+        if (getattr(to_qkv, 'bias', None) is None
+                and ops.linear_attention_block_supported(xn, spec, self._spec[id(to_out)], b_out, pre.fn.heads)):
+            return ops.linear_attention_block(xn, to_qkv.weight, spec, to_out.weight, b_out, self._spec[id(to_out)],
+                                              ops.stash_grad(x, sk), pre.fn.heads)
         if getattr(to_qkv, 'bias', None) is None and ops.linear_attention_fused_supported(xn, spec, pre.fn.heads):
             a = ops.linear_attention_fused(xn, to_qkv.weight, spec, pre.fn.heads)
         else:
```

New measurement: 7020 (median of 6 runs). 6.8% higher.
